# trzy/FasterRCNN

Measured on AMD Instinct MI355X. Metric: images/sec (600x1000) Faster-RCNN VGG-16 inference, higher is better.
Workload: dtype f32 (float32 tensors and accumulation; 15 GEMM layers in the f32x3 split-operand emulation = two fp16 terms per block-scaled operand, three fp16 MFMAs per product; 0 in f32x6 = three bf16 terms, six bf16 MFMAs; the other 2 on exact-f32 MFMA; strict exact-f32 everywhere: config.strict_f32_images_per_

## Files before the change

fasterrcnn_amd/_native.py:

```python
import ctypes as C
import os

_HERE = os.path.dirname(os.path.abspath(__file__))
LIB_PATH = os.environ.get("FRCNN_LIB_PATH") or os.path.join(_HERE, "csrc", "libfrcnn_hip.so")

OK = 0
ABI_VERSION = 21
ERRORS = {0: "FRCNN_OK", -1: "FRCNN_EINVAL", -2: "FRCNN_EHIP", -3: "FRCNN_ENOMEM",
          -4: "FRCNN_EUNSUPPORTED", -5: "FRCNN_ENODEVICE"}
RELU = 1
POOL2 = 2
NUM_KCLASS = 11
KCLASS_NAMES = ("conv3x3_mfma", "conv3x3_c3", "linear_mfma", "proposals", "roi_pool", "other", "winograd_transforms",
                "winograd_gemm", "winograd_x6_transforms", "winograd_x6_gemm", "winograd_x3f")

SYMBOLS = (
    "frcnn_abi_version", "frcnn_error_string", "frcnn_last_hip_error", "frcnn_device_count",
    "frcnn_anchors", "frcnn_pack_conv3x3", "frcnn_pack_conv3x3_c3", "frcnn_pack_fc_chw_to_hwc",
    "frcnn_pack_stack_rows", "frcnn_conv3x3_c3", "frcnn_conv3x3_c3_cmax", "frcnn_conv3x3_workspace_bytes", "frcnn_conv3x3_nhwc",
    "frcnn_maxpool2x2_nhwc",
    "frcnn_linear_workspace_bytes", "frcnn_linear", "frcnn_softmax_rows", "frcnn_rpn_proposals",
    "frcnn_nms", "frcnn_roi_pool", "frcnn_roi_pool_x3t", "frcnn_detections", "frcnn_ctx_create", "frcnn_ctx_create_proposals", "frcnn_ctx_destroy",
    "frcnn_ctx_bytes", "frcnn_vgg16_forward", "frcnn_ctx_tensor", "frcnn_ctx_timing_enable",
    "frcnn_ctx_timing_read",
    "frcnn_output_block_layout", "frcnn_stream_depend", "frcnn_ctx_submit_stats", "frcnn_predict_submit", "frcnn_streams_share_queue",
    "frcnn_fold_bn_pack", "frcnn_conv_workspace_bytes", "frcnn_conv_nhwc", "frcnn_conv_nhwc_math", "frcnn_conv_nhwc_x3g", "frcnn_conv_nhwc_x3g_tickets", "frcnn_pack_conv_x3g_weights", "frcnn_x3_saturation_events", "frcnn_tensor_absmax", "frcnn_conv7x7_s2_c3",
    "frcnn_maxpool3x3_s2_nhwc", "frcnn_spatial_mean_nhwc", "frcnn_resnet_forward", "frcnn_rpn_targets",
    "frcnn_preprocess_workspace_bytes", "frcnn_preprocess",
    "frcnn_conv3x3_uses_winograd", "frcnn_resnet_block_uses_winograd", "frcnn_pack_conv3x3_winograd",
    "frcnn_pack_conv3x3_winograd_taps", "frcnn_conv3x3_winograd_workspace_bytes",
    "frcnn_conv3x3_nhwc_winograd",
    "frcnn_conv3x3_uses_winograd_fused", "frcnn_resnet_block_uses_winograd_fused", "frcnn_pack_conv3x3_winograd_fused", "frcnn_pack_conv3x3_winograd_fused_taps",
    "frcnn_conv3x3_nhwc_winograd_fused",
    "frcnn_roi_align", "frcnn_roi_align_backward",
    "frcnn_x6t_record_bytes", "frcnn_split_rows_x6t", "frcnn_gemm_x6t_workspace_bytes", "frcnn_gemm_x6t", "frcnn_split_pixels_x6t", "frcnn_split_patches3x3_x6t",
    "frcnn_conv3x3_uses_winograd_x6", "frcnn_conv3x3_winograd_x6_pack_bytes", "frcnn_pack_conv3x3_winograd_x6",
    "frcnn_conv3x3_winograd_x6_workspace_bytes", "frcnn_conv3x3_nhwc_winograd_x6",
    "frcnn_pixel_absmax", "frcnn_split_pixels_x3t", "frcnn_split_patches3x3_x3t",
    "frcnn_x3t_blob_bytes", "frcnn_pack_rows_x3t", "frcnn_conv3x3_winograd_x3_pack_bytes", "frcnn_pack_conv3x3_winograd_x3",
    "frcnn_conv3x3_winograd_x3_workspace_bytes", "frcnn_conv3x3_nhwc_winograd_x3",
    "frcnn_conv3x3_winograd_x3_fused_workspace_bytes", "frcnn_conv3x3_nhwc_winograd_x3_fused", "frcnn_conv3x3_nhwc_winograd_x3_chain",
    "frcnn_x3t_record_bytes", "frcnn_rows_scale_x3t", "frcnn_split_rows_x3t", "frcnn_gemm_x3t_workspace_bytes", "frcnn_gemm_x3t",
    "frcnn_conv3x3_nhwc_winograd_fused_maps", "frcnn_ctx_create_backbone", "frcnn_resnet_backbone", "frcnn_resnet_forward_features", "frcnn_resnet_rpn_roipool", "frcnn_ctx_create_head", "frcnn_resnet_head",
    "frcnn_label_proposals", "frcnn_gather_rows", "frcnn_rpn_loss", "frcnn_detector_loss",
    "frcnn_gemm_tn_math", "frcnn_conv3x3_wgrad_math", "frcnn_conv_wgrad_math", "frcnn_bottleneck_backward_workspace_bytes", "frcnn_bottleneck_backward",
    "frcnn_gemm_tn_workspace_bytes", "frcnn_gemm_tn", "frcnn_conv3x3_wgrad_workspace_bytes", "frcnn_conv3x3_wgrad",
    "frcnn_pack_conv3x3_dgrad", "frcnn_relu_backward", "frcnn_dropout", "frcnn_dropout_relu_backward", "frcnn_add_inplace", "frcnn_maxpool2x2_backward",
    "frcnn_roi_pool_backward_workspace_bytes", "frcnn_roi_pool_backward", "frcnn_transpose", "frcnn_sgd_step", "frcnn_sgd_step_fold",
    "frcnn_conv_wgrad_workspace_bytes", "frcnn_conv_wgrad", "frcnn_conv_dgrad_workspace_bytes", "frcnn_conv_dgrad", "frcnn_conv_dgrad_math",
    "frcnn_pack_conv_dgrad", "frcnn_scale_rows", "frcnn_bn_scale_shift", "frcnn_spatial_mean_backward",
    "frcnn_ops_roi_align", "frcnn_ops_roi_align_backward", "frcnn_ops_roi_pool", "frcnn_ops_roi_pool_backward",
    "frcnn_ops_nms_workspace_bytes", "frcnn_ops_nms",
    "frcnn_ops_ms_roi_align", "frcnn_ops_ms_roi_align_workspace_bytes", "frcnn_ops_ms_roi_align_backward",
    "frcnn_ops_half_run", "frcnn_ops_roi_align_16", "frcnn_ops_roi_align_backward_16", "frcnn_ops_roi_pool_16",
    "frcnn_ops_roi_pool_backward_16", "frcnn_ops_ms_roi_align_16", "frcnn_ops_ms_roi_align_backward_16",
    "frcnn_ops_ps_roi_pool", "frcnn_ops_ps_roi_pool_backward", "frcnn_ops_ps_roi_align", "frcnn_ops_ps_roi_align_backward",
    "frcnn_ops_ps_roi_pool_16", "frcnn_ops_ps_roi_pool_backward_16", "frcnn_ops_ps_roi_align_16", "frcnn_ops_ps_roi_align_backward_16",
    "frcnn_ops_deform_workspace_bytes", "frcnn_ops_deform_forward", "frcnn_ops_deform_backward_columns", "frcnn_ops_deform_backward_offset",
    "frcnn_ops_deform_input_plan", "frcnn_ops_deform_backward_input", "frcnn_ops_deform_backward_weight",
    "frcnn_ops_deform_workspace_bytes_16", "frcnn_ops_deform_forward_16", "frcnn_ops_deform_backward_columns_16",
    "frcnn_ops_deform_backward_offset_16", "frcnn_ops_deform_input_plan_16", "frcnn_ops_deform_backward_input_16",
    "frcnn_ops_deform_backward_weight_16",
    "frcnn_ops_deform_roi_pool_cull_list", "frcnn_ops_deform_roi_pool_workspace_bytes", "frcnn_ops_deform_roi_pool",
    "frcnn_ops_deform_roi_pool_backward", "frcnn_ops_deform_roi_pool_16", "frcnn_ops_deform_roi_pool_backward_16",
    "frcnn_ops_box_iou_rotated", "frcnn_ops_nms_rotated", "frcnn_ops_roi_align_rotated_cull_list", "frcnn_ops_roi_align_rotated",
    "frcnn_ops_roi_align_rotated_backward", "frcnn_ops_roi_align_rotated_16", "frcnn_ops_roi_align_rotated_backward_16",
    "frcnn_ops_diff_iou_rotated", "frcnn_ops_diff_iou_rotated_backward",
    "frcnn_ops_convex_iou_tile_rows", "frcnn_ops_convex_iou", "frcnn_ops_convex_giou", "frcnn_ops_min_area_polygons",
    "frcnn_ops_soft_nms_block_threads", "frcnn_ops_soft_nms_lds_boxes", "frcnn_ops_soft_nms_max_boxes", "frcnn_ops_soft_nms_workspace_bytes",
    "frcnn_ops_soft_nms",
    "frcnn_ops_carafe_max_kernel", "frcnn_ops_carafe_channel_chunk", "frcnn_ops_carafe_tile_width", "frcnn_ops_carafe_tile_height",
    "frcnn_ops_carafe", "frcnn_ops_carafe_backward", "frcnn_ops_carafe_16", "frcnn_ops_carafe_backward_16",
    "frcnn_ops_msda_max_levels", "frcnn_ops_msda_max_points", "frcnn_ops_msda_max_channels", "frcnn_ops_msda_block_items",
    "frcnn_ops_msda_segment", "frcnn_ops_msda_workspace_bytes", "frcnn_ops_msda_forward", "frcnn_ops_msda_backward_loc", "frcnn_ops_msda_plan",
    "frcnn_ops_msda_backward_value", "frcnn_ops_msda_forward_16", "frcnn_ops_msda_backward_loc_16", "frcnn_ops_msda_backward_value_16",
    "frcnn_ops_prroi_pool_cull_list", "frcnn_ops_prroi_pool_workspace_bytes", "frcnn_ops_prroi_pool", "frcnn_ops_prroi_pool_backward",
    "frcnn_ops_prroi_pool_16", "frcnn_ops_prroi_pool_backward_16",
    "frcnn_ops_dcnv3_max_kernel", "frcnn_ops_dcnv3_max_channels", "frcnn_ops_dcnv3_block_items", "frcnn_ops_dcnv3_workspace_bytes",
    "frcnn_ops_dcnv3_forward", "frcnn_ops_dcnv3_backward_offset", "frcnn_ops_dcnv3_plan", "frcnn_ops_dcnv3_backward_input",
    "frcnn_ops_dcnv3_forward_16", "frcnn_ops_dcnv3_backward_offset_16", "frcnn_ops_dcnv3_backward_input_16",
    "frcnn_ops_dcnv4_record", "frcnn_ops_dcnv4_block_items", "frcnn_ops_dcnv4_workspace_bytes",
    "frcnn_ops_dcnv4_forward", "frcnn_ops_dcnv4_backward_offset_mask", "frcnn_ops_dcnv4_plan", "frcnn_ops_dcnv4_backward_input",
    "frcnn_ops_dcnv4_forward_16", "frcnn_ops_dcnv4_backward_offset_mask_16", "frcnn_ops_dcnv4_backward_input_16",
    "frcnn_ops_border_align_cull_list", "frcnn_ops_border_align", "frcnn_ops_border_align_backward", "frcnn_ops_border_align_16",
    "frcnn_ops_border_align_backward_16",
    "frcnn_ops_riroi_align_rotated_max_orientations", "frcnn_ops_riroi_align_rotated", "frcnn_ops_riroi_align_rotated_backward",
    "frcnn_ops_riroi_align_rotated_16", "frcnn_ops_riroi_align_rotated_backward_16",
    "frcnn_ops_rotated_feature_align", "frcnn_ops_rotated_feature_align_plan", "frcnn_ops_rotated_feature_align_backward",
    "frcnn_ops_rotated_feature_align_16", "frcnn_ops_rotated_feature_align_backward_16",
)


class FrcnnError(RuntimeError):
    def __init__(self, code, where, detail=""):
        self.code = code
        super().__init__("%s failed: %s (%d)%s" % (where, ERRORS.get(code, "?"), code,
                                                   (": " + detail) if detail else ""))


class VGG16Weights(C.Structure):
    _fields_ = [
        ("conv_w", C.c_void_p * 13), ("conv_b", C.c_void_p * 13),
        ("rpn_conv_w", C.c_void_p), ("rpn_conv_b", C.c_void_p),
        ("rpn_head_w", C.c_void_p), ("rpn_head_b", C.c_void_p),
# ... 190 lines not shown
    "frcnn_ops_convex_giou": (C.c_int, [_vp, _vp, _i, _vp, _vp, _vp]),
    "frcnn_ops_min_area_polygons": (C.c_int, [_vp, _i, _vp, _vp]),
    "frcnn_ops_soft_nms_block_threads": (C.c_int, []),
    "frcnn_ops_soft_nms_lds_boxes": (C.c_int, []),
    "frcnn_ops_soft_nms_max_boxes": (C.c_int, []),
    "frcnn_ops_soft_nms_workspace_bytes": (C.c_size_t, [_i]),
    "frcnn_ops_soft_nms": (C.c_int, [_vp, _vp, _vp, _vp, _i, _f, _f, _f, _i, _i, _vp, _vp, _vp, _sz, _vp]),
    "frcnn_ops_carafe_max_kernel": (C.c_int, []),
    "frcnn_ops_carafe_channel_chunk": (C.c_int, []),
    "frcnn_ops_carafe_tile_width": (C.c_int, []),
    "frcnn_ops_carafe_tile_height": (C.c_int, []),
    "frcnn_ops_carafe": (C.c_int, [_vp, _vp, _i, _i, _i, _i, _i, _i, _i, _vp, _vp]),
    "frcnn_ops_carafe_backward": (C.c_int, [_vp, _vp, _vp, _i, _i, _i, _i, _i, _i, _i, _vp, _vp, _vp]),
    "frcnn_ops_carafe_16": (C.c_int, [_i, _vp, _vp, _i, _i, _i, _i, _i, _i, _i, _vp, _vp]),
    "frcnn_ops_carafe_backward_16": (C.c_int, [_i, _vp, _vp, _vp, _i, _i, _i, _i, _i, _i, _i, _vp, _vp, _vp]),
    "frcnn_ops_msda_max_levels": (C.c_int, []),
    "frcnn_ops_msda_max_points": (C.c_int, []),
    "frcnn_ops_msda_max_channels": (C.c_int, []),
    "frcnn_ops_msda_block_items": (C.c_int, [_i, _i, _i, _i]),
    "frcnn_ops_msda_segment": (C.c_int, []),
    "frcnn_ops_msda_workspace_bytes": (C.c_size_t, [_i, _i, _i, _i, _i, _i, _i]),
    "frcnn_ops_msda_forward": (C.c_int, [_vp, _vp, _vp, _vp, _vp, _i, _i, _i, _i, _i, _i, _i, _vp, _vp]),
    "frcnn_ops_msda_backward_loc": (C.c_int, [_vp, _vp, _vp, _vp, _vp, _vp, _i, _i, _i, _i, _i, _i, _i, _vp, _vp, _vp]),
    "frcnn_ops_msda_plan": (C.c_int, [_vp, _vp, _vp, _vp, _i, _i, _i, _i, _i, _i, _vp, _vp, _vp]),
    "frcnn_ops_msda_backward_value": (C.c_int, [_vp, _vp, _vp, _vp, _i, _i, _i, _i, _i, _i, _i, _vp, _vp, _sz, _vp]),
    "frcnn_ops_msda_forward_16": (C.c_int, [_i, _vp, _vp, _vp, _vp, _vp, _i, _i, _i, _i, _i, _i, _i, _vp, _vp]),
    "frcnn_ops_msda_backward_loc_16": (C.c_int, [_i, _vp, _vp, _vp, _vp, _vp, _vp, _i, _i, _i, _i, _i, _i, _i, _vp, _vp, _vp]),
    "frcnn_ops_msda_backward_value_16": (C.c_int, [_i, _vp, _vp, _vp, _vp, _i, _i, _i, _i, _i, _i, _i, _vp, _vp, _sz, _vp]),
    "frcnn_ops_prroi_pool_cull_list": (C.c_int, []),
    "frcnn_ops_prroi_pool_workspace_bytes": (C.c_size_t, [_i, _i, _i]),
    "frcnn_ops_prroi_pool": (C.c_int, [_vp, _i, _i, _i, _i, _vp, _i, _i, _i, _f, _vp, _vp]),
    "frcnn_ops_prroi_pool_backward": (C.c_int, [_vp, _vp, _i, _i, _i, _i, _i, _i, _i, _f, _vp, _vp, _vp, _vp, _sz, _vp]),
    "frcnn_ops_prroi_pool_16": (C.c_int, [_i, _vp, _i, _i, _i, _i, _vp, _i, _i, _i, _f, _vp, _vp]),
    "frcnn_ops_prroi_pool_backward_16": (C.c_int, [_i, _vp, _vp, _i, _i, _i, _i, _i, _i, _i, _f, _vp, _vp, _vp, _vp, _sz, _vp]),
    "frcnn_ops_border_align_cull_list": (C.c_int, []),
    "frcnn_ops_border_align": (C.c_int, [_vp, _i, _i, _i, _i, _vp, _i, _i, _vp, _vp, _vp]),
    "frcnn_ops_border_align_backward": (C.c_int, [_vp, _i, _i, _i, _i, _i, _i, _vp, _vp, _vp, _vp]),
    "frcnn_ops_border_align_16": (C.c_int, [_i, _vp, _i, _i, _i, _i, _vp, _i, _i, _vp, _vp, _vp]),
    "frcnn_ops_border_align_backward_16": (C.c_int, [_i, _vp, _i, _i, _i, _i, _i, _i, _vp, _vp, _vp, _vp]),
    "frcnn_ops_rotated_feature_align": (C.c_int, [_vp, _vp, _i, _i, _i, _i, _f, _i, _vp, _vp]),
    "frcnn_ops_rotated_feature_align_plan": (C.c_int, [_vp, _i, _i, _i, _f, _i, _vp, _vp, _vp]),
    "frcnn_ops_rotated_feature_align_backward": (C.c_int, [_vp, _vp, _vp, _vp, _i, _i, _i, _i, _i, _vp, _vp]),
    "frcnn_ops_rotated_feature_align_16": (C.c_int, [_i, _vp, _vp, _i, _i, _i, _i, _f, _i, _vp, _vp]),
    "frcnn_ops_rotated_feature_align_backward_16": (C.c_int, [_i, _vp, _vp, _vp, _vp, _i, _i, _i, _i, _i, _vp, _vp]),
    "frcnn_ops_dcnv3_max_kernel": (C.c_int, []),
    "frcnn_ops_dcnv3_max_channels": (C.c_int, []),
    "frcnn_ops_dcnv3_block_items": (C.c_int, [_i, _i, _i, _i]),
    "frcnn_ops_dcnv3_workspace_bytes": (C.c_size_t, [_i] * 13),
    "frcnn_ops_dcnv3_forward": (C.c_int, [_vp, _vp, _vp] + [_i] * 13 + [_f, _vp, _vp]),
    "frcnn_ops_dcnv3_backward_offset": (C.c_int, [_vp, _vp, _vp, _vp] + [_i] * 13 + [_f, _vp, _vp, _vp]),
    "frcnn_ops_dcnv3_plan": (C.c_int, [_vp, _vp] + [_i] * 12 + [_f, _vp, _vp, _vp]),
    "frcnn_ops_dcnv3_backward_input": (C.c_int, [_vp, _vp, _vp, _vp] + [_i] * 13 + [_vp, _vp, _sz, _vp]),
    "frcnn_ops_dcnv3_forward_16": (C.c_int, [_i, _vp, _vp, _vp] + [_i] * 13 + [_f, _vp, _vp]),
    "frcnn_ops_dcnv3_backward_offset_16": (C.c_int, [_i, _vp, _vp, _vp, _vp] + [_i] * 13 + [_f, _vp, _vp, _vp]),
    "frcnn_ops_dcnv3_backward_input_16": (C.c_int, [_i, _vp, _vp, _vp, _vp] + [_i] * 13 + [_vp, _vp, _sz, _vp]),
    "frcnn_ops_dcnv4_record": (C.c_int, [_i, _i, _i, _i]),
    "frcnn_ops_dcnv4_block_items": (C.c_int, [_i, _i, _i, _i, _i]),
    "frcnn_ops_dcnv4_workspace_bytes": (C.c_size_t, [_i] * 14),
    "frcnn_ops_dcnv4_forward": (C.c_int, [_vp, _vp] + [_i] * 13 + [_f, _i, _vp, _vp]),
    "frcnn_ops_dcnv4_backward_offset_mask": (C.c_int, [_vp, _vp, _vp] + [_i] * 13 + [_f, _i, _vp, _vp]),
    "frcnn_ops_dcnv4_plan": (C.c_int, [_vp] + [_i] * 12 + [_f, _i, _vp, _vp, _vp]),
    "frcnn_ops_dcnv4_backward_input": (C.c_int, [_vp, _vp, _vp, _vp] + [_i] * 14 + [_vp, _vp, _sz, _vp]),
    "frcnn_ops_dcnv4_forward_16": (C.c_int, [_i, _vp, _vp] + [_i] * 13 + [_f, _i, _vp, _vp]),
    "frcnn_ops_dcnv4_backward_offset_mask_16": (C.c_int, [_i, _vp, _vp, _vp] + [_i] * 13 + [_f, _i, _vp, _vp]),
    "frcnn_ops_dcnv4_backward_input_16": (C.c_int, [_i, _vp, _vp, _vp, _vp] + [_i] * 14 + [_vp, _vp, _sz, _vp]),
    "frcnn_x6t_record_bytes": (C.c_size_t, [_i, _i]),
    "frcnn_split_rows_x6t": (C.c_int, [_vp, _i, _sz, _vp, _i, _i, _i, _i, _vp]),
    "frcnn_gemm_x6t_workspace_bytes": (C.c_size_t, [_i, _i, _i, _i]),
    "frcnn_gemm_x6t": (C.c_int, [_vp, _i, _sz, _vp, _i, _sz, _vp, _vp, _vp, _i, _sz, _i, _i, _i, _i, _u, _vp, _sz, _vp]),
    "frcnn_split_pixels_x6t": (C.c_int, [_vp, _vp, _i, _i, _i, _i, _i, _i, _vp]),
    "frcnn_conv3x3_uses_winograd_x6": (C.c_int, [_i, _i]),
    "frcnn_conv3x3_winograd_x6_pack_bytes": (C.c_size_t, [_i, _i]),
    "frcnn_pack_conv3x3_winograd_x6": (C.c_int, [_vp, _vp, _vp, _i, _i, _vp]),
    "frcnn_conv3x3_winograd_x6_workspace_bytes": (C.c_size_t, [_i, _i, _i, _i, _i]),
    "frcnn_conv3x3_nhwc_winograd_x6": (C.c_int, [_vp, _vp, _vp, _vp, _i, _i, _i, _i, _i, _u, _vp, _sz, _vp]),
    "frcnn_split_patches3x3_x6t": (C.c_int, [_vp, _vp, _i, _i, _i, _i, _i, _i, _vp]),
    "frcnn_conv3x3_uses_winograd_fused": (C.c_int, [_i, _i]),
    "frcnn_resnet_block_uses_winograd_fused": (C.c_int, [_i, _i, _i]),
    "frcnn_pack_conv3x3_winograd_fused": (C.c_int, [_vp, _vp, _vp, _i, _i, _vp]),
    "frcnn_pack_conv3x3_winograd_fused_taps": (C.c_int, [_vp, _vp, _i, _i, _i, _vp]),
    "frcnn_conv3x3_nhwc_winograd_fused": (C.c_int, [_vp, _vp, _vp, _vp, _i, _i, _i, _i, _u, _vp]),
    "frcnn_linear_workspace_bytes": (C.c_size_t, [_i, _i, _i]),
    "frcnn_linear": (C.c_int, [_vp, _i, _vp, _vp, _vp, _i, _i, _i, _i, _u, _vp, _sz, _vp]),
    "frcnn_softmax_rows": (C.c_int, [_vp, _i, _vp, _i, _i, _vp]),
    "frcnn_rpn_proposals": (C.c_int, [_vp, _vp, _i, _vp, _vp, _i, _i, _i, _i, _i, _i, _f, _f,
                                      _vp, _vp, _vp, _vp, _vp]),
    "frcnn_nms": (C.c_int, [_vp, _vp, _vp, _i, _f, _i, _vp, _vp, _vp]),
    "frcnn_roi_pool": (C.c_int, [_vp, _i, _i, _i, _vp, _vp, _i, _i, _f, _vp, _vp]),
    "frcnn_roi_pool_x3t": (C.c_int, [_vp, _i, _i, _i, _vp, _vp, _i, _i, _f, _vp, _vp, _vp, _i, _vp]),
    "frcnn_detections": (C.c_int, [_vp, _vp, _vp, _vp, _i, _i, _i, _i, _f, _f, _vp, _vp, _vp]),
    "frcnn_ctx_create": (C.c_int, [C.POINTER(C.c_void_p), _i, _i, _i]),
    "frcnn_ctx_create_proposals": (C.c_int, [C.POINTER(C.c_void_p), _i, _i]),
    "frcnn_ctx_destroy": (None, [_vp]),
    "frcnn_ctx_bytes": (C.c_size_t, [_vp]),
    "frcnn_vgg16_forward": (C.c_int, [_vp, C.POINTER(VGG16Weights), C.POINTER(ForwardParams), _vp, _i, _i,
                                      _vp, _vp, _vp, _vp, _vp, _vp, _vp]),
    "frcnn_ctx_tensor": (C.c_int, [_vp, _i, C.POINTER(C.c_void_p), C.POINTER(C.c_size_t)]),
    "frcnn_rpn_targets": (C.c_int, [_vp, _vp, _i, _vp, _i, C.c_double, C.c_double, _vp, _vp, _vp, _vp, _vp, _vp]),
    "frcnn_preprocess_workspace_bytes": (C.c_size_t, [_i, _i, _i, _i]),
    "frcnn_preprocess": (C.c_int, [_vp, _i, _i, _i, _i, _i, _i, _f, C.POINTER(C.c_float), C.POINTER(C.c_float), _vp, _vp,
                                   _vp, _sz, _vp]),
    "frcnn_fold_bn_pack": (C.c_int, [_vp, _vp, _vp, _vp, _vp, _f, _i, _i, _i, _vp, _vp, _vp]),
    "frcnn_conv_workspace_bytes": (C.c_size_t, [_i, _i, _i, _i, _i, _i, _i, _i]),
    "frcnn_conv_nhwc": (C.c_int, [_vp, _vp, _vp, _vp, _vp, _i, _i, _i, _i, _i, _i, _i, _i, _u, _vp, _sz, _vp]),
    "frcnn_x3_saturation_events": (C.c_int, [C.POINTER(C.c_ulonglong)]),
    "frcnn_conv_nhwc_math": (C.c_int, [_vp, _vp, _vp, _vp, _vp, _i, _i, _i, _i, _i, _i, _i, _i, _u, _i, _vp, _sz, _vp]),
    "frcnn_conv_nhwc_x3g": (C.c_int, [_vp, _vp, _vp, _vp, _vp, _i, _i, _i, _i, _i, _i, _i, _i, _u, _vp, _vp, _vp, _vp, _sz, _vp]),
    "frcnn_conv_nhwc_x3g_tickets": (C.c_int, [_vp, _vp, _vp, _vp, _vp, _i, _i, _i, _i, _i, _i, _i, _i, _u, _vp, _vp, _vp, _vp, _sz, _vp, _vp]),
    "frcnn_pack_conv_x3g_weights": (C.c_int, [_vp, _vp, _vp, _i, _i, _i, _vp]),
    "frcnn_tensor_absmax": (C.c_int, [_vp, C.c_longlong, _vp, _vp]),
    "frcnn_conv7x7_s2_c3": (C.c_int, [_vp, _vp, _vp, _vp, _i, _i, _i, _u, _vp]),
    "frcnn_maxpool3x3_s2_nhwc": (C.c_int, [_vp, _vp, _i, _i, _i, _vp]),
    "frcnn_spatial_mean_nhwc": (C.c_int, [_vp, _vp, _i, _i, _i, _i, _vp]),
    "frcnn_resnet_forward": (C.c_int, [_vp, C.POINTER(ResNetWeights), C.POINTER(ForwardParams), _vp, _i, _i,
                                       _vp, _vp, _vp, _vp, _vp, _vp, _vp]),
    "frcnn_resnet_forward_features": (C.c_int, [_vp, C.POINTER(ResNetWeights), C.POINTER(ForwardParams), _vp, _i, _i,
                                                _vp, _vp, _vp, _vp, _vp, _vp, _vp]),
    "frcnn_resnet_backbone": (C.c_int, [_vp, C.POINTER(ResNetWeights), C.POINTER(ForwardParams), _vp, _i, _i, _i, _vp, _vp]),
    "frcnn_pixel_absmax": (C.c_int, [_vp, _vp, C.c_longlong, _i, _vp]),
    "frcnn_split_pixels_x3t": (C.c_int, [_vp, _vp, _vp, _vp, _i, _i, _i, _i, _i, _i, _vp]),
    "frcnn_split_patches3x3_x3t": (C.c_int, [_vp, _vp, _vp, _vp, _i, _i, _i, _i, _i, _i, _vp]),
    "frcnn_x3t_blob_bytes": (C.c_size_t, [_i, _i, _i]),
    "frcnn_pack_rows_x3t": (C.c_int, [_vp, _i, _sz, _vp, _i, _i, _i, _i, _vp]),
    "frcnn_conv3x3_winograd_x3_pack_bytes": (C.c_size_t, [_i, _i]),
    "frcnn_pack_conv3x3_winograd_x3": (C.c_int, [_vp, _vp, _i, _i, _vp]),
    "frcnn_conv3x3_winograd_x3_workspace_bytes": (C.c_size_t, [_i, _i, _i, _i, _i]),
    "frcnn_conv3x3_nhwc_winograd_x3": (C.c_int, [_vp, _vp, _vp, _vp, _i, _i, _i, _i, _i, _u, _vp, _sz, _vp]),
    "frcnn_conv3x3_winograd_x3_fused_workspace_bytes": (C.c_size_t, [_i, _i, _i]),
    "frcnn_conv3x3_nhwc_winograd_x3_fused": (C.c_int, [_vp, _vp, _vp, _vp, _i, _i, _i, _i, _i, _u, _vp, _sz, _vp]),
    "frcnn_conv3x3_nhwc_winograd_x3_chain": (C.c_int, [_vp, _vp, _vp, _vp, _i, _i, _i, _i, _i, _u, _i, _vp, _sz, _vp, _vp, _vp]),
    "frcnn_x3t_record_bytes": (C.c_size_t, [_i, _i]),
    "frcnn_rows_scale_x3t": (C.c_int, [_vp, _i, _sz, _vp, _i, _i, _i, _i, _vp]),
    "frcnn_split_rows_x3t": (C.c_int, [_vp, _i, _sz, _vp, _vp, _i, _i, _i, _i, _vp]),
    "frcnn_gemm_x3t_workspace_bytes": (C.c_size_t, [_i, _i, _i, _i]),
    "frcnn_gemm_x3t": (C.c_int, [_vp, _vp, _i, _sz, _sz, _vp, _vp, _i, _sz, _sz, _vp, _vp, _vp, _i, _sz, _i, _i, _i, _i, _u, _vp, _sz, _vp]),
    "frcnn_ctx_create_backbone": (C.c_int, [C.POINTER(C.c_void_p), _i, _i, _i]),
    "frcnn_ctx_create_head": (C.c_int, [C.POINTER(C.c_void_p), _i]),
    "frcnn_resnet_rpn_roipool": (C.c_int, [_vp, C.POINTER(ResNetWeights), C.POINTER(ForwardParams), _vp, _i, _i, _vp, _vp, _vp, _vp, _vp, _vp]),
    "frcnn_resnet_head": (C.c_int, [_vp, C.POINTER(ResNetWeights), C.POINTER(ForwardParams), _vp, _i, _vp, _vp, _vp]),
    "frcnn_conv3x3_nhwc_winograd_fused_maps": (C.c_int, [_vp, _vp, _vp, _vp, _i, _i, _i, _i, _i, _u, _vp]),
    "frcnn_label_proposals": (C.c_int, [_vp, _vp, _i, _vp, _vp, _i, _i, _f, _f, C.POINTER(C.c_float), C.POINTER(C.c_float),
                                        _vp, _vp, _vp, _vp, _vp, _vp]),
    "frcnn_gather_rows": (C.c_int, [_vp, _vp, _i, _i, _vp, _vp]),
    "frcnn_rpn_loss": (C.c_int, [_vp, _i, _i, _vp, _i, _vp, _vp, _vp, _vp]),
    "frcnn_detector_loss": (C.c_int, [_vp, _vp, _vp, _vp, _i, _i, _vp, _vp, _i, _vp]),
    "frcnn_gemm_tn_workspace_bytes": (C.c_size_t, [_i, _i, _i]),
    "frcnn_gemm_tn": (C.c_int, [_vp, _i, _vp, _i, _vp, _i, _i, _i, _i, _vp, _sz, _vp]),
    "frcnn_gemm_tn_math": (C.c_int, [_vp, _i, _vp, _i, _vp, _i, _i, _i, _i, _i, _vp, _sz, _vp]),
    "frcnn_conv3x3_wgrad_math": (C.c_int, [_vp, _vp, _vp, _i, _i, _i, _i, _i, _vp, _sz, _vp]),
    "frcnn_conv_wgrad_math": (C.c_int, [_vp, _vp, _vp, _i, _i, _i, _i, _i, _i, _i, _i, _i, _vp, _sz, _vp]),
    "frcnn_bottleneck_backward_workspace_bytes": (C.c_int, [_vp, _vp, _vp, _vp, _i, _i, _i, _i, _i, C.POINTER(C.c_size_t), C.POINTER(C.c_size_t)]),
    "frcnn_bottleneck_backward": (C.c_int, [_vp, _vp, _vp, _vp, _vp, _vp, _vp, _vp, _vp, _vp, _vp, _vp, _vp, _i, _i, _i, _i, _i, _i, _vp, _sz, _vp, _sz,
                                            _vp, _vp]),
    "frcnn_conv3x3_wgrad_workspace_bytes": (C.c_size_t, [_i, _i, _i, _i]),
    "frcnn_conv3x3_wgrad": (C.c_int, [_vp, _vp, _vp, _i, _i, _i, _i, _vp, _sz, _vp]),
    "frcnn_pack_conv3x3_dgrad": (C.c_int, [_vp, _vp, _i, _i, _vp]),
    "frcnn_conv_wgrad_workspace_bytes": (C.c_size_t, [_i] * 8),
    "frcnn_conv_wgrad": (C.c_int, [_vp, _vp, _vp, _i, _i, _i, _i, _i, _i, _i, _i, _vp, _sz, _vp]),
    "frcnn_conv_dgrad_workspace_bytes": (C.c_size_t, [_i] * 8),
    "frcnn_conv_dgrad": (C.c_int, [_vp, _vp, _vp, _vp, _i, _i, _i, _i, _i, _i, _i, _i, _vp, _sz, _vp]),
    "frcnn_conv_dgrad_math": (C.c_int, [_vp, _vp, _vp, _vp, _i, _i, _i, _i, _i, _i, _i, _i, _i, _vp, _sz, _vp]),
    "frcnn_pack_conv_dgrad": (C.c_int, [_vp, _vp, _i, _i, _i, _vp]),
    "frcnn_scale_rows": (C.c_int, [_vp, _vp, _vp, _i, _i, _i, _vp]),
    "frcnn_bn_scale_shift": (C.c_int, [_vp, _vp, _vp, _vp, _f, _i, _vp, _vp, _vp]),
    "frcnn_spatial_mean_backward": (C.c_int, [_vp, _vp, _i, _i, _i, _i, _vp]),
    "frcnn_relu_backward": (C.c_int, [_vp, _vp, _sz, _vp]),
# ... 87 lines not shown
```

fasterrcnn_amd/csrc/api.hip:

```cpp
#include "common.h"
#include <algorithm>
#include <cmath>
#include <cstring>
#include <initializer_list>
#include <string>
#include <vector>
#include <new>

namespace frcnn {

static thread_local std::string g_hip_error;
void set_hip_error(hipError_t e) { g_hip_error = hipGetErrorString(e); }

static size_t align_up(size_t v, size_t a) { return (v + a - 1) / a * a; }

struct EventRec { int cls; hipEvent_t start, stop; };

struct Scratch {
    void* p = nullptr;
    size_t bytes = 0;
    int reserve(size_t want, hipStream_t s, bool zero)
    {
        if (want <= bytes) return FRCNN_OK;
        if (p) { FRCNN_HIP_TRY(hipStreamSynchronize(s)); release(); }
// ... 467 lines not shown

int frcnn_conv_nhwc_math(const float* d_x, const float* d_wp, const float* d_bias, const float* d_residual, float* d_y,
                         int N, int H, int W, int cin, int cout, int ksize, int stride, int pad, unsigned flags, int math,
                         void* d_ws, size_t ws_bytes, void* stream)
{
    if (!d_x || !d_wp || !d_bias || !d_y) return FRCNN_EINVAL;
    if (flags & FRCNN_POOL2) return FRCNN_EUNSUPPORTED;
    return launch_conv_gather(d_x, d_wp, d_bias, d_residual, d_y, N, H, W, cin, cout, ksize, stride, pad, flags,
                              d_ws, ws_bytes, as_stream(stream), math);
}

int frcnn_x3_saturation_events(unsigned long long* out)
{
    if (!out) return FRCNN_EINVAL;
    const unsigned* c = x3_saturation_counter();
    *out = c ? (unsigned long long)*reinterpret_cast<const volatile unsigned*>(c) : 0ull;
    return FRCNN_OK;
}

int frcnn_conv_nhwc_x3g(const float* d_x, const float* d_wp, const float* d_bias, const float* d_residual, float* d_y,
                        int N, int H, int W, int cin, int cout, int ksize, int stride, int pad, unsigned flags,
                        const float* d_xmax, const float* d_wmax, float* d_ymax, void* d_ws, size_t ws_bytes, void* stream)
{
    if (!d_x || !d_wp || !d_bias || !d_y || !d_xmax || !d_wmax) return FRCNN_EINVAL;
    if (flags & FRCNN_POOL2) return FRCNN_EUNSUPPORTED;
    const GatherX3 x3{d_xmax, d_wmax, d_ymax, nullptr, (flags & FRCNN_X3G_WSPLIT) != 0};
    return launch_conv_gather(d_x, d_wp, d_bias, d_residual, d_y, N, H, W, cin, cout, ksize, stride, pad, flags,
                              d_ws, ws_bytes, as_stream(stream), FRCNN_CONV_F32X3G, &x3);
}

int frcnn_pack_conv_x3g_weights(const float* d_wp, const float* d_wmax, void* d_out, int taps, int cout, int cin, void* stream)
{
    if (taps < 1 || cout < 1) return FRCNN_EINVAL;
    return launch_pack_x3g_weights(d_wp, d_wmax, d_out, (long long)taps * cout, cin, as_stream(stream));
}

int frcnn_conv_nhwc_x3g_tickets(const float* d_x, const float* d_wp, const float* d_bias, const float* d_residual, float* d_y,
                                int N, int H, int W, int cin, int cout, int ksize, int stride, int pad, unsigned flags,
                                const float* d_xmax, const float* d_wmax, float* d_ymax, void* d_ws, size_t ws_bytes,
                                unsigned* d_tile_counters, void* stream)
{
    static_assert(FRCNN_X3G_TILE_COUNTERS == GX_TILE_COUNTERS, "one bound on both sides of the ABI");
    if (!d_x || !d_wp || !d_bias || !d_y || !d_xmax || !d_wmax || !d_tile_counters) return FRCNN_EINVAL;
    if (flags & FRCNN_POOL2) return FRCNN_EUNSUPPORTED;
    const GatherX3 x3{d_xmax, d_wmax, d_ymax, d_tile_counters, (flags & FRCNN_X3G_WSPLIT) != 0};
    return launch_conv_gather(d_x, d_wp, d_bias, d_residual, d_y, N, H, W, cin, cout, ksize, stride, pad, flags,
                              d_ws, ws_bytes, as_stream(stream), FRCNN_CONV_F32X3G, &x3);
}

int frcnn_tensor_absmax(const float* d_x, long long n, float* d_out, void* stream)
{
    if (!d_x || !d_out) return FRCNN_EINVAL;
    return launch_tensor_absmax(d_x, n, d_out, as_stream(stream));
}

int frcnn_conv7x7_s2_c3(const float* d_x, const float* d_wp, const float* d_bias, float* d_y, int H, int W,
                        int cout, unsigned flags, void* stream)
{
    if (!d_x || !d_wp || !d_bias || !d_y) return FRCNN_EINVAL;
    return launch_conv7x7_s2_c3(d_x, d_wp, d_bias, d_y, H, W, cout, flags, as_stream(stream));
}

int frcnn_maxpool3x3_s2_nhwc(const float* d_x, float* d_y, int H, int W, int c, void* stream)
{
    if (!d_x || !d_y) return FRCNN_EINVAL;
    return launch_maxpool3x3_s2(d_x, d_y, H, W, c, as_stream(stream));
}

int frcnn_spatial_mean_nhwc(const float* d_x, float* d_y, int N, int H, int W, int c, void* stream)
{
    if (!d_x || !d_y) return FRCNN_EINVAL;
    return launch_spatial_mean(d_x, d_y, N, H, W, c, as_stream(stream));
}

size_t frcnn_linear_workspace_bytes(int M, int N, int K) { return linear_workspace_bytes(M, N, K); }

int frcnn_linear(const float* d_a, int lda, const float* d_w, const float* d_bias, float* d_y, int ldy,
                 int M, int N, int K, unsigned flags, void* d_ws, size_t ws_bytes, void* stream)
{
    if (!d_a || !d_w || !d_bias || !d_y) return FRCNN_EINVAL;
    return launch_linear(d_a, lda, d_w, d_bias, d_y, ldy, M, N, K, flags, d_ws, ws_bytes, as_stream(stream));
}

int frcnn_softmax_rows(const float* d_x, int ldx, float* d_y, int M, int ncls, void* stream)
{
    if (!d_x || !d_y) return FRCNN_EINVAL;
    return launch_softmax_rows(d_x, ldx, d_y, M, ncls, as_stream(stream));
}

int frcnn_rpn_proposals(frcnn_ctx* ctx, const float* d_head, int ld_head, const float* d_anchor_map,
                        const float* d_valid_map, int fh, int fw, int image_h, int image_w, int pre_nms,
                        int post_nms, float nms_threshold, float min_side, float* d_scores,
                        int32_t* d_sorted_idx, float* d_props, int32_t* d_counts, void* stream)
{
    if (!ctx || !d_head || !d_anchor_map || !d_scores || !d_sorted_idx || !d_props || !d_counts) return FRCNN_EINVAL;
    FRCNN_HIP_TRY(hipMemsetAsync(d_counts, 0, 4 * sizeof(int32_t), as_stream(stream)));
    return launch_rpn_proposals(ctx->ps, d_head, ld_head, d_anchor_map, d_valid_map, fh, fw, image_h, image_w,
                                pre_nms, post_nms, nms_threshold, min_side, d_scores, d_sorted_idx, d_props,
                                d_counts, as_stream(stream));
}

int frcnn_nms(frcnn_ctx* ctx, const float* d_boxes, const float* d_scores, int n, float threshold,
              int max_keep, int32_t* d_keep, int32_t* d_n_keep, void* stream)
{
    if (!ctx || !d_boxes || !d_scores || !d_keep || !d_n_keep) return FRCNN_EINVAL;
    return launch_nms(ctx->ps, d_boxes, d_scores, n, threshold, max_keep, d_keep, d_n_keep, as_stream(stream));
}

int frcnn_roi_pool(const float* d_fm, int fh, int fw, int c, const float* d_rois, const int32_t* d_n_rois,
                   int max_rois, int pooled, float spatial_scale, float* d_out, void* stream)
{
    if (!d_fm || !d_rois || !d_n_rois || !d_out) return FRCNN_EINVAL;
    return launch_roi_pool(d_fm, fh, fw, c, d_rois, d_n_rois, max_rois, pooled, spatial_scale, d_out,
                           as_stream(stream));
}

int frcnn_roi_pool_x3t(const float* d_fm, int fh, int fw, int c, const float* d_rois, const int32_t* d_n_rois, int max_rois, int pooled,
                       float spatial_scale, float* d_cmax, float* d_inv_scale, void* d_rec, int rec_rows, void* stream)
{
    if (!d_fm || !d_rois || !d_n_rois || !d_cmax || !d_inv_scale || !d_rec) return FRCNN_EINVAL;
    return launch_roi_pool_x3t(d_fm, fh, fw, c, d_rois, d_n_rois, max_rois, pooled, spatial_scale, d_cmax, d_inv_scale, d_rec, rec_rows,
                               as_stream(stream));
}

int frcnn_roi_align(const float* d_fm, int fh, int fw, int c, const float* d_rois, const int32_t* d_n_rois, int max_rois,
                    int pooled, float spatial_scale, int sampling_ratio, int aligned, float* d_out, void* stream)
{
    if (!d_fm || !d_rois || !d_n_rois || !d_out) return FRCNN_EINVAL;
    return launch_roi_align(d_fm, fh, fw, c, d_rois, d_n_rois, max_rois, pooled, spatial_scale, sampling_ratio, aligned, d_out,
                            as_stream(stream));
}

int frcnn_roi_align_backward(const float* d_rois, int n_rois, int fh, int fw, int c, int pooled, float spatial_scale,
                             int sampling_ratio, int aligned, const float* d_dout, float* d_dfm, int accumulate, void* stream)
{
    if (!d_dfm || (n_rois > 0 && (!d_rois || !d_dout))) return FRCNN_EINVAL;
    return launch_roi_align_backward(d_rois, n_rois, fh, fw, c, pooled, spatial_scale, sampling_ratio, aligned, d_dout, d_dfm,
                                     accumulate, as_stream(stream));
}

int frcnn_detections(const float* d_props, const float* d_classes, const float* d_deltas,
                     const int32_t* d_n_rois, int max_rois, int ncls, int image_h, int image_w,
                     float score_threshold, float nms_threshold, double* d_out, int32_t* d_out_cnt, void* stream)
{
    if (!d_props || !d_classes || !d_deltas || !d_n_rois || !d_out || !d_out_cnt) return FRCNN_EINVAL;
    return launch_detections(d_props, d_classes, d_deltas, d_n_rois, max_rois, ncls, image_h, image_w,
                             score_threshold, nms_threshold, d_out, d_out_cnt, as_stream(stream));
}

int frcnn_label_proposals(const float* d_props, const int32_t* d_n_props, int max_props,
                          const float* d_gt_boxes, const int32_t* d_gt_class_idx, int n_gt, int num_classes,
                          float min_background_iou, float min_object_iou,
                          const float box_delta_means[4], const float box_delta_stds[4],
                          float* d_out_props, int32_t* d_out_class_idx, float* d_out_gt_classes,
                          float* d_out_gt_box_deltas, int32_t* d_out_count, void* stream)
{
    if ((!d_props && max_props > 0) || !d_n_props || !d_gt_boxes || !d_gt_class_idx || !box_delta_means || !box_delta_stds ||
        !d_out_props || !d_out_class_idx || !d_out_gt_classes || !d_out_gt_box_deltas || !d_out_count)
        return FRCNN_EINVAL;
    if (!(min_background_iou < min_object_iou)) return FRCNN_EINVAL;
    return launch_label_proposals(d_props, d_n_props, max_props, d_gt_boxes, d_gt_class_idx, n_gt, num_classes,
                                  min_background_iou, min_object_iou, box_delta_means, box_delta_stds, d_out_props,
                                  d_out_class_idx, d_out_gt_classes, d_out_gt_box_deltas, d_out_count, as_stream(stream));
}

int frcnn_gather_rows(const float* d_src, const int32_t* d_idx, int n, int row_floats, float* d_dst, void* stream)
// ... 492 lines not shown
}

int run_wino_x6_layer(frcnn_ctx* c, const float* x, const void* urec, const float* b, float* y, int h, int w, int ci, int co,
                      unsigned flags, hipStream_t s, int N = 1)
{
    if (N == 1 && !conv3x3_uses_winograd_x6(ci, co)) return FRCNN_EINVAL;
    int r = ensure_wx_ws(c, conv3x3_winograd_x6_workspace_bytes(N, h, w, ci, co), s);
    if (r) return r;
    void *V = nullptr, *G = nullptr;
    float* M = nullptr;
    size_t gb = 0;
    r = winograd_x6_plan(N, h, w, ci, co, flags, c->wx_ws.p, c->wx_ws.bytes, &V, &M, &G, &gb);
    if (r) return r;
    { Scope _t(c, 8, s); r = launch_winograd_x6_input(x, V, N, h, w, ci, s); }
    if (r) return r;
    { Scope _g(c, 9, s); r = launch_winograd_x6_gemm(V, urec, M, N, h, w, ci, co, G, gb, s); }
    if (r) return r;
    Scope _o(c, 8, s);
    return launch_winograd_output(M, b, y, N, h, w, co, flags, s);
}

int run_wino_x3_layer(frcnn_ctx* c, const float* x, const void* ublob, const float* b, float* y, int h, int w, int ci, int co,
                      unsigned flags, hipStream_t s, int N = 1, const float* cmax_ready = nullptr, float* cmax_out = nullptr)
{
    if (N == 1 && !conv3x3_uses_winograd_x6(ci, co)) return FRCNN_EINVAL;
    int r = ensure_wx_ws(c, conv3x3_winograd_x3_workspace_bytes(N, h, w, ci, co), s);
    if (r) return r;
    void *V = nullptr, *G = nullptr;
    float *M = nullptr, *vinv = nullptr, *cmax = nullptr;
    size_t gb = 0;
    r = winograd_x3_plan(N, h, w, ci, co, flags, c->wx_ws.p, c->wx_ws.bytes, &V, &vinv, &cmax, &M, &G, &gb);
    if (r) return r;
    { Scope _t(c, 8, s); r = launch_winograd_x3_input(x, cmax, V, vinv, N, h, w, ci, s, cmax_ready); }
    if (r) return r;
    { Scope _g(c, 9, s); r = launch_winograd_x3_gemm(V, vinv, ublob, M, N, h, w, ci, co, G, gb, s); }
    if (r) return r;
    Scope _o(c, 8, s);
    return launch_winograd_output(M, b, y, N, h, w, co, flags, s, cmax_out);
}

int ensure_x3f_cmax(frcnn_ctx* c, size_t need, hipStream_t s)
{
    return c->x3f_cmax.reserve(3 * std::max(need, (size_t)c->max_h * c->max_w * sizeof(float)), s, false);
}
size_t x3f_cmax_bytes(const frcnn_ctx* c) { return c->x3f_cmax.bytes / 3; }
float* x3f_cmax_buffer(frcnn_ctx* c, int which) { return reinterpret_cast<float*>(static_cast<unsigned char*>(c->x3f_cmax.p) + (size_t)which * x3f_cmax_bytes(c)); }

int run_wino_x3f_layer(frcnn_ctx* c, const float* x, const void* ublob, const float* b, float* y, int h, int w, int ci, int co,
                       unsigned flags, hipStream_t s, const float* cmax_ready = nullptr, float* cmax_out = nullptr)
{
    int r = ensure_x3f_cmax(c, conv3x3_winograd_x3_fused_workspace_bytes(1, h, w), s);
    if (r) return r;
    Scope _w(c, 10, s);
    return launch_conv3x3_winograd_x3_fused(x, ublob, b, y, 1, h, w, ci, co, flags, x3f_cmax_buffer(c, 0), x3f_cmax_bytes(c), s, cmax_ready, cmax_out);
}

int run_wino_fused_layer(frcnn_ctx* c, bool , const float* x, const float* u, const float* b, float* y, int h, int w, int ci,
                         int co, unsigned flags, hipStream_t s, int n_maps = 1)
{
    Scope _w(c, 7, s);
    return launch_conv3x3_winograd_fused(x, u, b, y, h, w, ci, co, flags, s, n_maps);
}

struct BlocksTargetScope {
    explicit BlocksTargetScope(int t, int wino_rows = 0, int x6_tiles = 0) { conv3x3_set_blocks_target(t); linear_batched_set_tile(wino_rows); gemm_x6t_set_tiles(x6_tiles); }
    ~BlocksTargetScope() { conv3x3_set_blocks_target(0); linear_batched_set_tile(0); gemm_x6t_set_tiles(0); }
};

int check_forward_params(const frcnn_forward_params* p, int bad_math_mode)
{
    if ((p->winograd_x3_mask & ~p->winograd_x6_mask) != 0) return FRCNN_EINVAL;
    if (p->math_mode != FRCNN_MATH_F32 && p->math_mode != FRCNN_MATH_F32_WINOGRAD) return bad_math_mode;
    if ((p->roi_op != FRCNN_ROI_POOL && p->roi_op != FRCNN_ROI_ALIGN) || p->roi_sampling_ratio > 2) return FRCNN_EINVAL;
    if (p->conv_blocks_target < 0) return FRCNN_EINVAL;
    if (p->winograd_tile_rows != 0 && p->winograd_tile_rows != 64 && p->winograd_tile_rows != 128) return FRCNN_EINVAL;
    if (p->x6_gemm_tiles < 0 || p->x6_gemm_tiles > 2) return FRCNN_EINVAL;
    return FRCNN_OK;
}

int run_rpn_after_trunk(frcnn_ctx* c, const float* head_w, const float* head_b, const frcnn_forward_params* p, int H, int W, int fh, int fw,
                        int C, const float* d_anchor_map, const float* d_valid_map, float* d_props, int32_t* d_counts, hipStream_t s)
{
    int rc;
    STEP(2, launch_linear(c->rpn_trunk, C, head_w, head_b, c->rpn_head, 128, fh * fw, 45, C, 0u, c->lin_ws, c->lin_ws_bytes, s));
    const float* amap = d_anchor_map;
    const float* vmap = d_valid_map;
    if (!amap || !vmap) {
        if (c->anc_h != H || c->anc_w != W || c->anc_fh != fh || c->anc_fw != fw) {
            STEP(5, launch_anchors(H, W, fh, fw, 16, c->anchor_map, c->valid_map, s));
            c->anc_h = H; c->anc_w = W; c->anc_fh = fh; c->anc_fw = fw;
        }
        amap = c->anchor_map; vmap = c->valid_map;
    }
    FRCNN_HIP_TRY(hipMemsetAsync(d_counts, 0, 4 * sizeof(int32_t), s));
    STEP(3, launch_rpn_proposals(c->ps, c->rpn_head, 128, amap, p->allow_edge_proposals ? nullptr : vmap, fh, fw,
                                 H, W, p->pre_nms, p->post_nms, p->rpn_nms_threshold, p->min_side, c->scores,
                                 c->sorted_idx, d_props, d_counts, s));
    return FRCNN_OK;
}

int run_roi_f32(frcnn_ctx* c, const frcnn_forward_params* p, int fh, int fw, int C, const float* d_props, const int32_t* d_counts,
                float* dst, hipStream_t s)
{
    Scope _sc(c, 4, s);
    if (p->roi_op == FRCNN_ROI_ALIGN)
        return launch_roi_align(c->fm, fh, fw, C, d_props, d_counts + 2, p->post_nms, 7, 1.0f / 16.0f, p->roi_sampling_ratio, 0, dst, s);
    return launch_roi_pool(c->fm, fh, fw, C, d_props, d_counts + 2, p->post_nms, 7, 1.0f / 16.0f, dst, s);
}

int run_detector_heads(frcnn_ctx* c, const float* head_w, const float* head_b, int ncls, int V, int n_rois, float* d_classes,
                       float* d_deltas, hipStream_t s)
{
    int rc;
    const int nd = (ncls - 1) * 4;
    const int hld = cdiv(ncls + nd, 128) * 128;
    c->last_head_ld = hld;
    STEP(2, launch_linear(c->fc2_out, V, head_w, head_b, c->head_logits, hld, n_rois, ncls + nd, V, 0u, c->lin_ws, c->lin_ws_bytes, s));
    STEP(5, launch_head_finish(c->head_logits, hld, n_rois, ncls, nd, d_classes, d_deltas, s));
    return FRCNN_OK;
}
}

int frcnn_vgg16_forward(frcnn_ctx* c, const frcnn_vgg16_weights* w, const frcnn_forward_params* p,
                        const float* d_image, int H, int W, const float* d_anchor_map,
                        const float* d_valid_map, float* d_props, float* d_classes, float* d_deltas,
                        int32_t* d_counts, void* stream)
{
    if (!c || !w || !p || !d_image || !d_props || !d_classes || !d_deltas || !d_counts) return FRCNN_EINVAL;
    if (H < 16 || W < 16 || H > c->max_h || W > c->max_w) return FRCNN_EINVAL;
    if (p->post_nms < 1 || p->post_nms > c->max_rois || p->pre_nms < 1 || p->pre_nms > c->pre_cap) return FRCNN_EINVAL;
    if (w->num_classes < 2 || w->num_classes > FRCNN_MAX_NUM_CLASSES) return FRCNN_EUNSUPPORTED;
    for (int i = 0; i < 13; ++i) if (!w->conv_w[i] || !w->conv_b[i]) return FRCNN_EINVAL;
    if (!w->rpn_conv_w || !w->rpn_conv_b || !w->rpn_head_w || !w->rpn_head_b || !w->fc1_w || !w->fc1_b ||
        !w->fc2_w || !w->fc2_b || !w->head_w || !w->head_b)
        return FRCNN_EINVAL;
    hipStream_t s = as_stream(stream);
    const unsigned R = FRCNN_RELU, RP = FRCNN_RELU | FRCNN_POOL2;
    int rc = check_forward_params(p, FRCNN_EINVAL);
    if (rc) return rc;
    if (p->fc_math_mode != FRCNN_FC_F32 && p->fc_math_mode != FRCNN_FC_F32X6T && p->fc_math_mode != FRCNN_FC_F32X3T) return FRCNN_EINVAL;
    BlocksTargetScope target_scope(p->conv_blocks_target, p->winograd_tile_rows, p->x6_gemm_tiles);
    const bool wino = p->math_mode == FRCNN_MATH_F32_WINOGRAD;
    if (p->winograd_x6_mask != 0 && (!wino || (p->winograd_x6_mask & ~0x3FFE) != 0)) return FRCNN_EINVAL;
    if (p->winograd_x3f_mask != 0 && (!wino || (p->winograd_x3f_mask & ~0x3FFE) != 0 || (p->winograd_x3f_mask & p->winograd_x6_mask) != 0)) return FRCNN_EINVAL;
    int layer_index = 0;
    const float* cmax_ready = nullptr;
    size_t cmax_used = 0, cmax_cleared = 0;
    if (wino && ((p->winograd_x3f_mask | (p->winograd_x3_mask & p->winograd_x6_mask)) & 0x1FFE) != 0) {
        int r0 = ensure_x3f_cmax(c, (size_t)H * W * sizeof(float), s);
        if (r0) return r0;
        static const int co_of[13] = {0, 64, 128, 128, 256, 256, 256, 512, 512, 512, 512, 512, 512};
        static const bool pool_of[13] = {false, true, false, true, false, false, true, false, false, true, false, false, false};
        size_t want = 0;
        int eh = H, ew = W;
        for (int li = 1; li <= 12; ++li) {
            const bool f3 = ((p->winograd_x3f_mask >> li) & 1) != 0;
            const bool t3 = !f3 && ((p->winograd_x6_mask >> li) & 1) && ((p->winograd_x3_mask >> li) & 1);
            const unsigned efl = FRCNN_RELU | (pool_of[li] ? FRCNN_POOL2 : 0u);
            if (pool_of[li]) { eh /= 2; ew /= 2; }
            if ((f3 || t3) && (f3 || winograd_output_emits_cmax(co_of[li], efl))) want += ((size_t)eh * ew + 63) & ~(size_t)63;
        }
        if (want > 2 * x3f_cmax_bytes(c) / sizeof(float)) return FRCNN_EINVAL;
        cmax_cleared = want;
        if (want) FRCNN_HIP_TRY(hipMemsetAsync(x3f_cmax_buffer(c, 1), 0, cmax_cleared * sizeof(float), s));
    }
    auto conv3 = [&](const float* xin, const float* wgt, const float* bs, float* yout, int hh, int ww, int ci, int co,
                     unsigned fl) -> int {
        ++layer_index;
        const float* in_cmax = cmax_ready;
        cmax_ready = nullptr;
        const bool is_x3f = wino && ((p->winograd_x3f_mask >> layer_index) & 1);
        const bool is_x3 = wino && !is_x3f && ((p->winograd_x6_mask >> layer_index) & 1) && ((p->winograd_x3_mask >> layer_index) & 1);
        float* out_cmax = nullptr;
        if ((is_x3f || is_x3) && layer_index != FRCNN_X6_RPN_TRUNK_BIT && (fl & FRCNN_RELU) && (is_x3f || winograd_output_emits_cmax(co, fl))) {
            const int oh = (fl & FRCNN_POOL2) ? hh / 2 : hh, ow = (fl & FRCNN_POOL2) ? ww / 2 : ww;
            const size_t need = ((size_t)oh * ow + 63) & ~(size_t)63;
            out_cmax = x3f_cmax_buffer(c, 1) + cmax_used;
            cmax_used += need;
            if (cmax_used > cmax_cleared) return FRCNN_EINVAL;
        }
        int r1;
        if (is_x3f)
            r1 = run_wino_x3f_layer(c, xin, wgt, bs, yout, hh, ww, ci, co, fl, s, in_cmax, out_cmax);
        else if (is_x3)
            r1 = run_wino_x3_layer(c, xin, wgt, bs, yout, hh, ww, ci, co, fl, s, 1, in_cmax, out_cmax);
        else if (wino && ((p->winograd_x6_mask >> layer_index) & 1))
            r1 = run_wino_x6_layer(c, xin, wgt, bs, yout, hh, ww, ci, co, fl, s);
        else
            r1 = -9999;
        if (r1 != -9999) {
            if (r1 == FRCNN_OK) cmax_ready = out_cmax;
            return r1;
        }
        if (wino && conv3x3_uses_winograd_fused(ci, co)) {
            return run_wino_fused_layer(c, p->conv_blocks_target == 0, xin, wgt, bs, yout, hh, ww, ci, co, fl, s);
        }
        Scope _d(c, 0, s);
        return launch_conv3x3_nhwc(xin, wgt, bs, yout, hh, ww, ci, co, fl, c->conv_ws, c->conv_ws_bytes, s);
    };
#define CONV(call) do { rc = (call); } while (0); if (rc) return rc

// ... 610 lines not shown
```

fasterrcnn_amd/csrc/common.h:

```cpp
#pragma once
#include <hip/hip_runtime.h>
#include <stdint.h>
#include <stddef.h>
#include <stdlib.h>
#include "../../include/frcnn_hip.h"

typedef float f32x4  __attribute__((ext_vector_type(4)));
typedef float f32x16 __attribute__((ext_vector_type(16)));

inline const char* frcnn_knob(const char* name)
{
#ifdef FRCNN_EXPERIMENT_KNOBS
    return getenv(name);
#else
    (void)name;
    return nullptr;
#endif
}

namespace frcnn {

void set_hip_error(hipError_t e);

inline int check_launch() {
    hipError_t e = hipGetLastError();
    if (e != hipSuccess) { set_hip_error(e); return FRCNN_EHIP; }
    return FRCNN_OK;
}

#define FRCNN_HIP_TRY(expr)                                   \
    do {                                                      \
        hipError_t _e = (expr);                               \
        if (_e != hipSuccess) { ::frcnn::set_hip_error(_e); return FRCNN_EHIP; } \
    } while (0)

static inline int cdiv(int a, int b) { return (a + b - 1) / b; }

struct DeviceOnce { unsigned char done[64]; };
inline int set_max_dynamic_lds(DeviceOnce& once, const void* kern, size_t bytes)
{
    int dev = 0;
    FRCNN_HIP_TRY(hipGetDevice(&dev));
    if (dev < 0 || dev >= 64) return FRCNN_EINVAL;
    if (!once.done[dev]) {
        FRCNN_HIP_TRY(hipFuncSetAttribute(kern, hipFuncAttributeMaxDynamicSharedMemorySize, (int)bytes));
        once.done[dev] = 1;
    }
    return FRCNN_OK;
}
#define FRCNN_MAX_LDS_ONCE(kern, bytes)                                                                  \
    do {                                                                                                 \
        static ::frcnn::DeviceOnce _once = {};                                                           \
        const int _rc = ::frcnn::set_max_dynamic_lds(_once, reinterpret_cast<const void*>(kern), (bytes)); \
        if (_rc) return _rc;                                                                             \
    } while (0)

static inline bool conv3x3_uses_winograd(int cin, int cout) { return cin >= 128 && cout >= 256 && cin % 16 == 0 && cout % 128 == 0; }
static inline bool resnet_block_uses_winograd(int width, int stride) { return stride == 1 && width >= 256 && width % 128 == 0; }

struct KernelTimer;

}

namespace frcnn {

int launch_anchors(int image_h, int image_w, int fh, int fw, int feature_pixels,
                   float* anchor_map, float* valid_map, hipStream_t s);

int launch_pack_conv3x3(const float* w, float* wp, int cout, int cin, hipStream_t s);
int launch_pack_conv3x3_c3(const float* w, float* wp, int cout, hipStream_t s);
int launch_pack_fc_chw_to_hwc(const float* w, float* wp, int out_f, int c, int phw, hipStream_t s);
int launch_pack_stack_rows(const float* w1, const float* b1, int n1, const float* w2, const float* b2,
                           int n2, int k, int n_pad, float* wo, float* bo, hipStream_t s);

int launch_conv3x3_c3(const float* x, const float* wp, const float* b, float* y, int H, int W,
                      int cout, unsigned flags, hipStream_t s, float* cmax_out = nullptr);
size_t conv3x3_workspace_bytes(int H, int W, int cin, int cout);
int conv3x3_blocks_target();
void conv3x3_set_blocks_target(int target);
int launch_conv3x3_nhwc(const float* x, const float* wp, const float* b, float* y, int H, int W,
                        int cin, int cout, unsigned flags, void* ws, size_t ws_bytes, hipStream_t s);
int launch_maxpool2x2(const float* x, float* y, int H, int W, int c, hipStream_t s);

size_t conv_gather_workspace_bytes(int N, int H, int W, int cin, int cout, int R, int stride, int pad);
#define FRCNN_CONV_F32X3G 2
static constexpr int GX_TILE_COUNTERS = 16384;
struct GatherX3 { const float* xmax; const float* wmax; float* ymax; unsigned* tile_counters = nullptr; bool wsplit = false; bool trusted = false; };
int launch_pack_x3g_weights(const float* wp, const float* wmax, void* out, long long rows, int cin, hipStream_t s);
int launch_conv_gather(const float* x, const float* wp, const float* bias, const float* residual, float* y,
                       int N, int H, int W, int cin, int cout, int R, int stride, int pad, unsigned flags,
                       void* ws, size_t ws_bytes, hipStream_t s, int math = FRCNN_GRAD_F32, const GatherX3* x3 = nullptr);
unsigned* x3_saturation_counter();
int launch_tensor_absmax(const float* x, long long n, float* out, hipStream_t s);
int launch_conv7x7_s2_c3(const float* x, const float* wp, const float* b, float* y, int H, int W, int cout,
                         unsigned flags, hipStream_t s);
int launch_maxpool3x3_s2(const float* x, float* y, int H, int W, int c, hipStream_t s);
int launch_spatial_mean(const float* x, float* y, int N, int H, int W, int c, hipStream_t s);
int launch_fold_bn_pack(const float* w, const float* gamma, const float* beta, const float* mean, const float* var,
                        float eps, int cout, int cin, int ksize, float* wp, float* bp, hipStream_t s);

size_t linear_workspace_bytes(int M, int N, int K);
int launch_linear(const float* a, int lda, const float* w, const float* bias, float* y, int ldy,
                  int M, int N, int K, unsigned flags, void* ws, size_t ws_bytes, hipStream_t s);
int launch_linear_batched(const float* a, int lda, size_t a_stride, const float* w, size_t w_stride, float* y, int ldy,
                          size_t y_stride, int M, int N, int K, int batches, hipStream_t s);
void linear_batched_set_tile(int rows);
size_t conv3x3_winograd_workspace_bytes(int N, int H, int W, int cin, int cout);
int launch_pack_conv3x3_winograd(const float* w, const float* scale, float* u, int cout, int cin, hipStream_t s);
int launch_pack_conv3x3_winograd_taps(const float* wp, float* u, int cout, int cin, int data_gradient, hipStream_t s);
int launch_conv3x3_winograd(const float* x, const float* u, const float* b, float* y, int N, int H, int W, int cin, int cout,
                            unsigned flags, void* ws, size_t ws_bytes, hipStream_t s);
int winograd_plan(int N, int H, int W, int cin, int cout, unsigned flags, void* ws, size_t ws_bytes, float** V, float** M);
int launch_winograd_input(const float* x, float* V, int N, int H, int W, int cin, hipStream_t s);
int launch_winograd_gemm(const float* V, const float* u, float* M, int N, int H, int W, int cin, int cout, hipStream_t s);
int launch_winograd_output(const float* M, const float* b, float* y, int N, int H, int W, int cout, unsigned flags, hipStream_t s,
                           float* cmax_out = nullptr);
bool winograd_output_emits_cmax(int cout, unsigned flags);
static inline bool conv3x3_uses_winograd_fused(int cin, int cout) { return cin >= 64 && cin % 16 == 0 && cout >= 64 && cout % 64 == 0; }
static inline bool resnet_block_uses_winograd_fused(int n_maps, int width, int stride)
{
    return n_maps == 1 && stride == 1 && conv3x3_uses_winograd_fused(width, width);
}
bool conv3x3_winograd_fused_ok(int H, int W, int cin, int cout);
int launch_pack_conv3x3_winograd_fused(const float* w, const float* scale, float* u, int cout, int cin, hipStream_t s);
int launch_pack_conv3x3_winograd_fused_taps(const float* wp, float* u, int cout, int cin, int data_gradient, hipStream_t s);
int launch_conv3x3_winograd_fused(const float* x, const float* u, const float* b, float* y, int H, int W, int cin, int cout,
                                  unsigned flags, hipStream_t s, int n_maps = 1);
int gemm_x6t_row_tile(int M);
int gemm_x6t_col_tile(int N);
size_t x6t_record_bytes(int rows_padded, int K);
int launch_split_rows_x6t(const float* a, int lda, size_t a_batch_floats, void* rec, int R, int rows_padded, int K, int batches, hipStream_t s);
bool gemm_x6t_shape_ok(int M, int N, int K, int batches);
size_t gemm_x6t_workspace_bytes(int M, int N, int K, int batches);
void gemm_x6t_set_tiles(int mode);
int launch_gemm_x6t(const void* a_rec, int a_rows, size_t a_batch_bytes, const void* b_rec, int b_rows, size_t b_batch_bytes,
                    const float* bias, const float* residual, float* c, int ldc, size_t c_batch_floats, int M, int N, int K, int batches,
                    unsigned flags, void* ws, size_t ws_bytes, hipStream_t s, int tiles_mode = -1);
int launch_split_pixels_x6t(const float* x, void* rec, int N, int H, int W, int C, int stride, int rows_padded, hipStream_t s);
int gemm_x6t_get_tiles();
int launch_gemm_x6t_reduce(const float* ws, const float* bias, const float* residual, float* c, int ldc, size_t c_batch_floats, int M, int N,
                           int batches, int splits, int relu, hipStream_t s);
size_t x3t_record_bytes(int rows_padded, int K);
int launch_rows_scale_x3t(const float* a, int lda, size_t a_batch_floats, float* inv_scale, int R, int rows_padded, int K, int batches,
                          hipStream_t s);
int launch_split_rows_x3t(const float* a, int lda, size_t a_batch_floats, const float* inv_scale, void* rec, int R, int rows_padded, int K,
                          int batches, hipStream_t s);
int launch_split_pixels_x3t(const float* x, const float* cmax, void* rec, float* inv, int N, int H, int W, int C, int stride, int rows_padded,
                            hipStream_t s);
int launch_split_patches3x3_x3t(const float* x, const float* cmax, void* rec, float* inv, int N, int H, int W, int C, int stride,
                                int rows_padded, hipStream_t s);
size_t gemm_x3t_workspace_bytes(int M, int N, int K, int batches);
int launch_gemm_x3t(const void* a_rec, const float* a_inv, int a_rows, size_t a_batch_bytes, size_t a_inv_batch, const void* b_rec,
                    const float* b_inv, int b_rows, size_t b_batch_bytes, size_t b_inv_batch, const float* bias, const float* residual,
                    float* c, int ldc, size_t c_batch_floats, int M, int N, int K, int batches, unsigned flags, void* ws, size_t ws_bytes,
                    hipStream_t s, int tiles_mode = -1);
size_t x3t_blob_bytes(int rows_padded, int K, int batches);
int launch_pack_rows_x3t(const float* a, int lda, size_t a_batch_floats, void* blob, int R, int rows_padded, int K, int batches, hipStream_t s);
int launch_pixel_absmax(const float* x, float* cmax, long long pixels, int C, hipStream_t s);
size_t conv3x3_winograd_x3_pack_bytes(int cout, int cin);
int launch_pack_conv3x3_winograd_x3(const float* u_f32, void* ublob, int cout, int cin, hipStream_t s);
size_t conv3x3_winograd_x3_workspace_bytes(int N, int H, int W, int cin, int cout);
int winograd_x3_plan(int N, int H, int W, int cin, int cout, unsigned flags, void* ws, size_t ws_bytes, void** V, float** vinv, float** cmax,
                     float** M, void** G, size_t* g_bytes);
int launch_winograd_x3_input(const float* x, float* cmax, void* vrec, float* vinv, int N, int H, int W, int cin, hipStream_t s,
                             const float* cmax_ready = nullptr);
int launch_winograd_x3_gemm(const void* vrec, const float* vinv, const void* ublob, float* M, int N, int H, int W, int cin, int cout, void* gws,
                            size_t gws_bytes, hipStream_t s);
int launch_conv3x3_winograd_x3(const float* x, const void* ublob, const float* b, float* y, int N, int H, int W, int cin, int cout,
                               unsigned flags, void* ws, size_t ws_bytes, hipStream_t s,
                               const float* cmax_ready = nullptr, float* cmax_out = nullptr);
size_t conv3x3_winograd_x3_fused_workspace_bytes(int N, int H, int W);
int launch_conv3x3_winograd_x3_fused(const float* x, const void* ublob, const float* b, float* y, int N, int H, int W, int cin, int cout,
                                     unsigned flags, void* ws, size_t ws_bytes, hipStream_t s, const float* cmax_ready = nullptr,
                                     float* cmax_out = nullptr);
int launch_roi_pool_x3t(const float* fm, int fh, int fw, int c, const float* rois, const int32_t* n_rois, int max_rois, int pooled,
                        float scale, float* cmax, float* inv, void* rec, int rec_rows, hipStream_t s, bool cmax_ready = false);
bool conv3x3_uses_winograd_x6(int cin, int cout);
size_t conv3x3_winograd_x6_pack_bytes(int cout, int cin);
size_t conv3x3_winograd_x6_workspace_bytes(int N, int H, int W, int cin, int cout);
int launch_pack_conv3x3_winograd_x6(const float* w, const float* scale, void* urec, int cout, int cin, hipStream_t s);
int launch_winograd_x6_input(const float* x, void* vrec, int N, int H, int W, int cin, hipStream_t s);
int launch_winograd_x6_gemm(const void* vrec, const void* urec, float* M, int N, int H, int W, int cin, int cout, void* gws, size_t gws_bytes, hipStream_t s);
int winograd_x6_plan(int N, int H, int W, int cin, int cout, unsigned flags, void* ws, size_t ws_bytes, void** V, float** M, void** G, size_t* g_bytes);
int launch_conv3x3_winograd_x6(const float* x, const void* urec, const float* b, float* y, int N, int H, int W, int cin, int cout,
                               unsigned flags, void* ws, size_t ws_bytes, hipStream_t s);
int launch_split_patches3x3_x6t(const float* x, void* rec, int N, int H, int W, int C, int stride, int rows_padded, hipStream_t s);
int launch_softmax_rows(const float* x, int ldx, float* y, int M, int ncls, hipStream_t s);
int launch_head_finish(const float* x, int ldx, int M, int ncls, int ndelta, float* classes,
                       float* deltas, hipStream_t s);

struct ProposalScratch {
    unsigned long long* keys;
    float*    boxes_all;
    float*    cand_boxes;
    float*    cand_scores;
    unsigned long long* mask;
    int32_t*  keep;
    int       a_cap, pre_cap, post_cap;
};
size_t proposal_scratch_bytes(int a_cap, int pre_cap, int post_cap);
void   proposal_scratch_carve(ProposalScratch& ps, void* base, int a_cap, int pre_cap, int post_cap);

int launch_rpn_proposals(const ProposalScratch& ps, const float* head, int ld_head,
                         const float* anchor_map, const float* valid_map, int fh, int fw,
                         int image_h, int image_w, int pre_nms, int post_nms, float nms_thr,
                         float min_side, float* scores, int32_t* sorted_idx, float* props,
                         int32_t* counts, hipStream_t s);
int launch_nms(const ProposalScratch& ps, const float* boxes, const float* scores, int n, float thr,
               int max_keep, int32_t* keep, int32_t* n_keep, hipStream_t s);

int launch_roi_pool(const float* fm, int fh, int fw, int c, const float* rois, const int32_t* n_rois,
                    int max_rois, int pooled, float scale, float* out, hipStream_t s);
int launch_roi_pool_x6t(const float* fm, int fh, int fw, int c, const float* rois, const int32_t* n_rois,
                        int max_rois, int pooled, float scale, void* rec, int rec_rows, hipStream_t s);

int launch_roi_align(const float* fm, int fh, int fw, int c, const float* rois, const int32_t* n_rois, int max_rois, int pooled,
                     float scale, int sampling_ratio, int aligned, float* out, hipStream_t s);
int launch_roi_align_backward(const float* rois, int n_rois, int fh, int fw, int c, int pooled, float scale, int sampling_ratio,
                              int aligned, const float* dout, float* dfm, int accumulate, hipStream_t s);

int launch_rpn_targets(const float* anchor_map, const float* valid_map, int A, const float* gt, int M,
                       double obj_thr, double bg_thr, float* rpn_map, int32_t* obj_idx, int32_t* bg_idx,
                       int32_t* counts, void* ws, hipStream_t s);

size_t preprocess_workspace_bytes(int H, int W, int Ho, int Wo);
int launch_preprocess(const unsigned char* rgb, int H, int W, int Ho, int Wo, int bgr, int flip, float scaling,
                      const float* means, const float* stds, float* out, unsigned char* out_u8, void* ws,
                      size_t ws_bytes, hipStream_t s);

int launch_detections(const float* props, const float* classes, const float* deltas,
                      const int32_t* n_rois, int max_rois, int ncls, int image_h, int image_w,
                      float score_thr, float nms_thr, double* out, int32_t* out_cnt, hipStream_t s);

size_t gemm_tn_workspace_bytes(int M, int N, int R, int taps);
int launch_gemm_tn(const float* A, int lda, const float* B, int ldb, float* C, int ldc, int M, int N, int R,
                   void* ws, size_t ws_bytes, hipStream_t s, int math = FRCNN_GRAD_F32);
int launch_conv3x3_wgrad(const float* x, const float* dz, float* dwp, int H, int W, int cin, int cout,
                         void* ws, size_t ws_bytes, hipStream_t s, int math = FRCNN_GRAD_F32);
int gemm_nt16_splits(int M, int N, int R);
size_t gemm_nt16_workspace_bytes(int M, int N, int R);
int launch_gemm_nt16(int elem_type, const void* A, int lda, const void* B, int ldb, float* C, int ldc, int M, int N, int R, hipStream_t s);
int launch_gemm_nt16_split(int elem_type, const void* A, int lda, const void* B, int ldb, float* C, int ldc, int M, int N, int R,
                           int accumulate, void* ws, size_t ws_bytes, hipStream_t s);
int launch_gemm_nt16_nchw(int elem_type, const void* A, int lda, const void* B, int ldb, int M, int N, int R, const void* bias, void* out,
                          int P, int c_total, int c_base, hipStream_t s);
int launch_label_proposals(const float* props, const int32_t* n_props, int max_props, const float* gt,
                           const int32_t* gt_cls, int M, int ncls, float bg_thr, float obj_thr,
                           const float means[4], const float stds[4], float* out_props, int32_t* out_cls,
                           float* out_onehot, float* out_deltas, int32_t* out_count, hipStream_t s);
int launch_gather_rows(const float* src, const int32_t* idx, int n, int row_floats, float* dst, hipStream_t s);
int launch_rpn_loss(const float* head, int ld, int cells, const int32_t* sample, int n_sample, const float* rpn_map,
                    float* losses, float* d_head, hipStream_t s);
int launch_detector_loss(const float* classes, const float* deltas, const float* gt_onehot, const float* gt_deltas,
                         int S, int ncls, float* losses, float* d_logits, int ld, hipStream_t s);
int launch_relu_backward(float* dy, const float* y, size_t n, hipStream_t s);
int launch_dropout(float* x, size_t n, float p, float scale, const uint64_t* seed, uint32_t stream_id, uint32_t rank,
                   uint8_t* keep_out, hipStream_t s);
int launch_dropout_relu_backward(float* dy, const float* y, size_t n, float scale, hipStream_t s);
int launch_add_inplace(float* a, const float* b, size_t n, hipStream_t s);
int launch_maxpool2x2_backward(const float* x, const float* dy, float* dx, int H, int W, int C, hipStream_t s);
size_t roi_pool_backward_workspace_bytes(int n_rois, int pooled, int C);
int launch_roi_pool_backward(const float* fm, int fh, int fw, int C, const float* rois, int n_rois, int pooled,
                             float scale, const float* dout, float* dfm, int accumulate, void* ws, size_t ws_bytes,
                             hipStream_t s);
int launch_transpose(const float* x, int ldi, float* y, int ldo, int rows, int cols, hipStream_t s);
int launch_pack_conv3x3_dgrad(const float* wp, float* wd, int cout, int cin, hipStream_t s);
int launch_conv_wgrad(const float* x, const float* dz, float* dwp, int N, int H, int W, int cin, int cout, int ks, int stride,
                      int pad, void* ws, size_t ws_bytes, hipStream_t s, int math = FRCNN_GRAD_F32);
size_t conv_dgrad_workspace_bytes(int N, int H, int W, int cin, int cout, int R, int stride, int pad);
int launch_conv_dgrad(const float* dz, const float* wd, const float* residual, float* dx, int N, int H, int W, int cin,
                      int cout, int R, int stride, int pad, void* ws, size_t ws_bytes, hipStream_t s, int math = FRCNN_GRAD_F32);
int launch_pack_conv_dgrad(const float* wp, float* wd, int taps, int cout, int cin, hipStream_t s);
int launch_scale_rows(const float* src, const float* scale, float* dst, int taps, int cout, int cin, hipStream_t s);
int launch_bn_scale_shift(const float* gamma, const float* beta, const float* mean, const float* var, float eps, int c,
                          float* scale, float* shift, hipStream_t s);
int launch_spatial_mean_backward(const float* dy, float* dx, int N, int H, int W, int c, hipStream_t s);
int launch_sgd(float* w, const float* g, float* buf, size_t n, float lr, float momentum, float weight_decay, int first,
               hipStream_t s);
int launch_sgd_fold(float* w, const float* g, float* buf, size_t n, float lr, float momentum, float weight_decay, int first,
                    const float* scale, float* folded, int cout, int cin, hipStream_t s);

}
```

fasterrcnn_amd/csrc/linear.hip:

```cpp
#include "common.h"
#include <cstdlib>

namespace frcnn {

static constexpr int LLDK = 20;

template <int TM, int TN, int WM, int WN>
struct GemmCfg {
    static constexpr int BM = 32 * TM * WM;
    static constexpr int BN = 32 * TN * WN;
    static constexpr int THREADS = 64 * WM * WN;
    static constexpr int NA = (BM * 4 + THREADS - 1) / THREADS;
    static constexpr int NB = (BN * 4 + THREADS - 1) / THREADS;
    static constexpr int A_F = BM * LLDK;
    static constexpr int B_F = BN * LLDK;
    static constexpr size_t LDS_BYTES = (size_t)2 * (A_F + B_F) * sizeof(float);
    static_assert(THREADS == 256 || THREADS == 512, "4 or 8 waves per block");
};

struct BatchGeom { long long a_stride, w_stride, y_stride; int nblocks, mblocks, batches; };

template <int TM, int TN, int WM, int WN, bool BATCHED, int NSETS = 2>
__global__ __launch_bounds__(64 * WM * WN)
void linear_mfma_kernel(const float* __restrict__ a, int lda, const float* __restrict__ w,
// ... 150 lines not shown
            for (int s = 0; s < nst; ++s) stage(s, areg[0], breg[0]);
        }
    }

    const bool direct = (gridDim.z == 1);
    float* const dst = direct ? y : ws + (size_t)blockIdx.z * M * N;
    const int ldd = direct ? ldy : N;
#pragma unroll
    for (int j = 0; j < TN; ++j) {
        const int n = n0 + 32 * (TN * wn + j) + li;
        if (n >= N) continue;
        const float bv = (direct && bias != nullptr) ? bias[n] : 0.f;
#pragma unroll
        for (int i = 0; i < TM; ++i) {
#pragma unroll
            for (int r = 0; r < 16; ++r) {
                const int m = m0 + 32 * (TM * wm + i) + (r & 3) + 8 * (r >> 2) + 4 * lh;
                if (m < M) {
                    float v = acc[i][j][r] + bv;
                    if (direct && relu) v = fmaxf(v, 0.f);
                    dst[(size_t)m * ldd + n] = v;
                }
            }
        }
    }
}

__global__ __launch_bounds__(256)
void splitk_reduce_kernel(const float* __restrict__ ws, const float* __restrict__ bias,
                          float* __restrict__ y, int ldy, int M, int N, int splits, int relu)
{
    const size_t total = (size_t)M * N;
    for (size_t i = (size_t)blockIdx.x * 256 + threadIdx.x; i < total; i += (size_t)gridDim.x * 256) {
        const int n = (int)(i % N);
        const size_t m = i / N;
        float v = ws[i];
        for (int z = 1; z < splits; ++z) v += ws[(size_t)z * total + i];
        v += bias[n];
        if (relu) v = fmaxf(v, 0.f);
        y[m * ldy + n] = v;
    }
}

__global__ __launch_bounds__(256)
void softmax_rows_kernel(const float* __restrict__ x, int ldx, float* __restrict__ y, int M, int ncls)
{
    const int row = blockIdx.x * 4 + (threadIdx.x >> 6);
    const int lane = threadIdx.x & 63;
    if (row >= M) return;
    const float* xr = x + (size_t)row * ldx;
    const float v0 = lane < ncls ? xr[lane] : -INFINITY, v1 = lane + 64 < ncls ? xr[lane + 64] : -INFINITY;
    float mx = fmaxf(v0, v1);
#pragma unroll
    for (int o = 32; o > 0; o >>= 1) mx = fmaxf(mx, __shfl_xor(mx, o));
    const float e0 = lane < ncls ? expf(v0 - mx) : 0.f, e1 = lane + 64 < ncls ? expf(v1 - mx) : 0.f;
    double sum = (double)e0 + (double)e1;
#pragma unroll
    for (int o = 32; o > 0; o >>= 1) sum += __shfl_xor(sum, o);
    if (lane < ncls) y[(size_t)row * ncls + lane] = (float)((double)e0 / sum);
    if (lane + 64 < ncls) y[(size_t)row * ncls + lane + 64] = (float)((double)e1 / sum);
}

__global__ __launch_bounds__(256)
void head_finish_kernel(const float* __restrict__ x, int ldx, int M, int ncls, int ndelta,
                        float* __restrict__ classes, float* __restrict__ deltas)
{
    const int row = blockIdx.x * 4 + (threadIdx.x >> 6);
    const int lane = threadIdx.x & 63;
    if (row >= M) return;
    const float* xr = x + (size_t)row * ldx;
    const float v0 = lane < ncls ? xr[lane] : -INFINITY, v1 = lane + 64 < ncls ? xr[lane + 64] : -INFINITY;
    float mx = fmaxf(v0, v1);
#pragma unroll
    for (int o = 32; o > 0; o >>= 1) mx = fmaxf(mx, __shfl_xor(mx, o));
    const float e0 = lane < ncls ? expf(v0 - mx) : 0.f, e1 = lane + 64 < ncls ? expf(v1 - mx) : 0.f;
    float sum = e0 + e1;
#pragma unroll
    for (int o = 32; o > 0; o >>= 1) sum += __shfl_xor(sum, o);
    if (lane < ncls) classes[(size_t)row * ncls + lane] = e0 / sum;
    if (lane + 64 < ncls) classes[(size_t)row * ncls + lane + 64] = e1 / sum;
    for (int j = lane; j < ndelta; j += 64) deltas[(size_t)row * ndelta + j] = xr[ncls + j];
}

__global__ void pack_fc_chw_to_hwc_kernel(const float* __restrict__ w, float* __restrict__ wp,
                                          int out_f, int c, int hw)
{
    const size_t K = (size_t)c * hw;
    const size_t total = (size_t)out_f * K;
    for (size_t i = (size_t)blockIdx.x * 256 + threadIdx.x; i < total; i += (size_t)gridDim.x * 256) {
        const size_t o = i / K, kk = i % K;
        const int p = (int)(kk / c), ch = (int)(kk % c);
        wp[i] = w[o * K + (size_t)ch * hw + p];
    }
}

__global__ void pack_stack_rows_kernel(const float* __restrict__ w1, const float* __restrict__ b1, int n1,
                                       const float* __restrict__ w2, const float* __restrict__ b2, int n2,
                                       int k, int n_pad, float* __restrict__ wo, float* __restrict__ bo)
{
    const size_t total = (size_t)n_pad * k;
    for (size_t i = (size_t)blockIdx.x * 256 + threadIdx.x; i < total; i += (size_t)gridDim.x * 256) {
        const int row = (int)(i / k), col = (int)(i % k);
        float v = 0.f;
        if (row < n1) v = w1[(size_t)row * k + col];
        else if (row < n1 + n2) v = w2[(size_t)(row - n1) * k + col];
        wo[i] = v;
        if (col == 0) bo[row] = row < n1 ? b1[row] : (row < n1 + n2 ? b2[row - n1] : 0.f);
    }
}

struct LinearPlan { bool big; int mblocks, nblocks, splits, stages_per_split; };

static LinearPlan plan_linear(int M, int N, int K)
{
    LinearPlan p;
    p.big = (M <= 320) || (M % 320 == 0);
    const int bm = p.big ? 320 : 128;
    p.mblocks = cdiv(M, bm);
    p.nblocks = cdiv(N, 128);
    const int stages = K / 16;
    static int target = -1;
    if (target < 0) { const char* e = frcnn_knob("FRCNN_LINEAR_BLOCKS_TARGET"); target = e ? atoi(e) : 256; if (target < 1) target = 1; }
    int want = target / (p.mblocks * p.nblocks);
    int cap = stages / 8;
    if (cap < 1) cap = 1;
    if (want > cap) want = cap;
    if (want < 1) want = 1;
    p.stages_per_split = cdiv(stages, want);
    p.splits = cdiv(stages, p.stages_per_split);
    return p;
}

size_t linear_workspace_bytes(int M, int N, int K)
{
    if (M < 1 || N < 1 || K < 16) return 0;
    const LinearPlan p = plan_linear(M, N, K);
    return p.splits > 1 ? (size_t)p.splits * M * N * sizeof(float) : 0;
}

template <int TM, int TN, int WM, int WN>
static int launch_linear_cfg(const LinearPlan& p, const float* a, int lda, const float* w,
                             const float* bias, float* y, int ldy, float* ws, int M, int N, int K,
                             int relu, hipStream_t s)
{
    using C = GemmCfg<TM, TN, WM, WN>;
    auto kern = linear_mfma_kernel<TM, TN, WM, WN, false>;
    FRCNN_MAX_LDS_ONCE(kern, C::LDS_BYTES);
    dim3 grid(p.nblocks, p.mblocks, p.splits);
    hipLaunchKernelGGL(kern, grid, dim3(C::THREADS), C::LDS_BYTES, s, a, lda, w, bias, y, ldy, ws, M, N, K,
                       p.stages_per_split, relu, BatchGeom{0, 0, 0, 0, 0, 0});
    return check_launch();
}

template <int TM, int TN, int WM, int WN, int NSETS>
static int launch_linear_batched_cfg(const float* a, int lda, const float* w, float* y, int ldy, int M, int N, int K,
                                     const BatchGeom& bg, hipStream_t s)
{
    using C = GemmCfg<TM, TN, WM, WN>;
    auto kern = linear_mfma_kernel<TM, TN, WM, WN, true, NSETS>;
    FRCNN_MAX_LDS_ONCE(kern, C::LDS_BYTES);
    const long long total = (long long)bg.nblocks * bg.mblocks * bg.batches;
    if (total < 1 || total > 0x7fffffffLL) return FRCNN_EINVAL;
    hipLaunchKernelGGL(kern, dim3((unsigned)total), dim3(C::THREADS), C::LDS_BYTES, s, a, lda, w,
                       (const float*)nullptr, y, ldy, (float*)nullptr, M, N, K, K >> 4, 0, bg);
    return check_launch();
}

static thread_local int g_batched_tile = 0;
void linear_batched_set_tile(int rows) { g_batched_tile = rows; }

int launch_linear_batched(const float* a, int lda, size_t a_stride, const float* w, size_t w_stride, float* y, int ldy,
                          size_t y_stride, int M, int N, int K, int batches, hipStream_t s)
{
    if (M < 1 || N < 1 || K < 16 || K % 16 != 0 || lda % 4 != 0 || lda < K || ldy < N || batches < 1) return FRCNN_EINVAL;
    static int env_tile = -1;
    if (env_tile < 0) { const char* e = frcnn_knob("FRCNN_WINO_TILE"); env_tile = e ? atoi(e) : 0; }
    const int tile = env_tile ? env_tile : (g_batched_tile ? g_batched_tile : 64);
    BatchGeom bg{(long long)a_stride, (long long)w_stride, (long long)y_stride, cdiv(N, 128), cdiv(M, 128), batches};
    if (tile == 128) return launch_linear_batched_cfg<2, 2, 2, 2, 1>(a, lda, w, y, ldy, M, N, K, bg, s);
    bg.mblocks = cdiv(M, 64);
    return launch_linear_batched_cfg<1, 2, 2, 2, 1>(a, lda, w, y, ldy, M, N, K, bg, s);
}

int launch_linear(const float* a, int lda, const float* w, const float* bias, float* y, int ldy,
                  int M, int N, int K, unsigned flags, void* ws, size_t ws_bytes, hipStream_t s)
{
    if (M < 1 || N < 1 || K < 16 || K % 16 != 0 || lda % 4 != 0 || lda < K || ldy < N) return FRCNN_EINVAL;
    const LinearPlan p = plan_linear(M, N, K);
    const size_t need = p.splits > 1 ? (size_t)p.splits * M * N * sizeof(float) : 0;
    if (need > ws_bytes || (need > 0 && ws == nullptr)) return FRCNN_EINVAL;
    const int relu = (flags & FRCNN_RELU) ? 1 : 0;
    int rc = p.big ? launch_linear_cfg<5, 1, 2, 4>(p, a, lda, w, bias, y, ldy, (float*)ws, M, N, K, relu, s)
                   : launch_linear_cfg<2, 2, 2, 2>(p, a, lda, w, bias, y, ldy, (float*)ws, M, N, K, relu, s);
    if (rc != FRCNN_OK) return rc;
    if (p.splits > 1) {
        const size_t total = (size_t)M * N;
        int blocks = (int)((total + 255) / 256);
        if (blocks > 2048) blocks = 2048;
        hipLaunchKernelGGL(splitk_reduce_kernel, dim3(blocks), dim3(256), 0, s, (const float*)ws, bias,
                           y, ldy, M, N, p.splits, relu);
        rc = check_launch();
    }
    return rc;
}

int launch_softmax_rows(const float* x, int ldx, float* y, int M, int ncls, hipStream_t s)
{
    if (M < 1 || ncls < 1 || ncls > 128 || ldx < ncls) return FRCNN_EINVAL;
    hipLaunchKernelGGL(softmax_rows_kernel, dim3(cdiv(M, 4)), dim3(256), 0, s, x, ldx, y, M, ncls);
    return check_launch();
}

int launch_head_finish(const float* x, int ldx, int M, int ncls, int ndelta, float* classes,
                       float* deltas, hipStream_t s)
{
    if (M < 1 || ncls < 1 || ncls > 128 || ndelta < 0 || ldx < ncls + ndelta) return FRCNN_EINVAL;
    hipLaunchKernelGGL(head_finish_kernel, dim3(cdiv(M, 4)), dim3(256), 0, s, x, ldx, M, ncls, ndelta,
                       classes, deltas);
    return check_launch();
}

int launch_pack_fc_chw_to_hwc(const float* w, float* wp, int out_f, int c, int phw, hipStream_t s)
{
    if (out_f < 1 || c < 1 || phw < 1) return FRCNN_EINVAL;
    hipLaunchKernelGGL(pack_fc_chw_to_hwc_kernel, dim3(8192), dim3(256), 0, s, w, wp, out_f, c, phw);
    return check_launch();
}

int launch_pack_stack_rows(const float* w1, const float* b1, int n1, const float* w2, const float* b2,
                           int n2, int k, int n_pad, float* wo, float* bo, hipStream_t s)
{
    if (n1 < 0 || n2 < 0 || n1 + n2 > n_pad || k < 1) return FRCNN_EINVAL;
    const size_t total = (size_t)n_pad * k;
    int blocks = (int)((total + 255) / 256);
    if (blocks > 2048) blocks = 2048;
    hipLaunchKernelGGL(pack_stack_rows_kernel, dim3(blocks), dim3(256), 0, s, w1, b1, n1, w2, b2, n2, k,
                       n_pad, wo, bo);
    return check_launch();
}

}
```

fasterrcnn_amd/csrc/proposals.hip:

```cpp
#include "geometry.h"
#include <type_traits>

namespace frcnn {

typedef unsigned long long u64;

__device__ __forceinline__ unsigned ordered_bits(float f)
{
    const unsigned b = __float_as_uint(f);
    return (b & 0x80000000u) ? ~b : (b | 0x80000000u);
}
__device__ __forceinline__ float from_ordered_bits(unsigned o)
{
    const unsigned b = (o & 0x80000000u) ? (o & 0x7fffffffu) : ~o;
    return __uint_as_float(b);
}

__global__ __launch_bounds__(256)
void rpn_decode_kernel(const float* __restrict__ head, int ld, const float* __restrict__ anchors,
                       const float* __restrict__ valid, int A, float* __restrict__ scores,
                       f32x4* __restrict__ boxes_all, u64* __restrict__ keys)
{
    const int n = blockIdx.x * 256 + threadIdx.x;
    if (n >= A) return;
    const int pix = n / 9, k = n - pix * 9;
    const float* row = head + (size_t)pix * ld;
    const float logit = row[k];
    const float score = 1.0f / (1.0f + expf(-logit));
    const float dy = row[9 + 4 * k + 0], dx = row[9 + 4 * k + 1];
    const float dh = row[9 + 4 * k + 2], dw = row[9 + 4 * k + 3];
    const f32x4 a = reinterpret_cast<const f32x4*>(anchors)[n];
    const float cy = __fadd_rn(__fmul_rn(a[2], dy), a[0]);
    const float cx = __fadd_rn(__fmul_rn(a[3], dx), a[1]);
    const float h = __fmul_rn(a[2], expf(dh));
    const float w = __fmul_rn(a[3], expf(dw));
    const float hh = 0.5f * h, hw = 0.5f * w;
    f32x4 b;
    b[0] = cy - hh; b[1] = cx - hw; b[2] = cy + hh; b[3] = cx + hw;
    scores[n] = score;
    boxes_all[n] = b;
    const bool ok = (valid == nullptr) || (valid[n] > 0.f);
    keys[n] = ok ? (((u64)ordered_bits(score) << 32) | (u64)(unsigned)(n + 1)) : 0ull;
}

__global__ __launch_bounds__(256)
void nms_keys_kernel(const float* __restrict__ scores, int n, u64* __restrict__ keys)
{
    const int i = blockIdx.x * 256 + threadIdx.x;
    if (i >= n) return;
    const float f = scores[i];
    const unsigned hi = f != f ? 0u : ordered_bits(f == 0.f ? 0.f : f);
    keys[i] = ((u64)hi << 32) | (u64)(0xFFFFFFFFu - (unsigned)i);
}

__device__ __forceinline__ u64 shfl_xor_u64(u64 v, int lane_mask)
{
    const unsigned lo = __shfl_xor((unsigned)(v & 0xFFFFFFFFull), lane_mask);
    const unsigned hi = __shfl_xor((unsigned)(v >> 32), lane_mask);
    return ((u64)hi << 32) | lo;
}

__device__ __forceinline__ u64 bitonic_pick(u64 mine, u64 other, int g, int j, int k)
{
    const bool keep_max = (((g & k) == 0) == ((g & j) == 0));
    const bool other_bigger = other > mine;
    return (keep_max == other_bigger) ? other : mine;
}

template <int PER, int J>
__device__ __forceinline__ void bitonic_inthread(u64 (&e)[PER], int base, int k)
{
#pragma unroll
    for (int r = 0; r < PER; ++r) {
        if ((r & J) == 0) {
            const u64 a = e[r], b = e[r | J];
            e[r] = bitonic_pick(a, b, base + r, J, k);
            e[r | J] = bitonic_pick(b, a, base + (r | J), J, k);
        }
    }
}

template <int PER>
__device__ void bitonic_sort_regs(u64* buf, int tid)
{
    constexpr int N = 1024 * PER;
    u64 e[PER];
    const int base = tid * PER;
#pragma unroll
    for (int r = 0; r < PER; ++r) e[r] = buf[base + r];
    for (int k = 2; k <= N; k <<= 1) {
        for (int j = k >> 1; j > 0; j >>= 1) {
            if (j >= 64 * PER) {
#pragma unroll
                for (int r = 0; r < PER; ++r) buf[base + r] = e[r];
                __syncthreads();
#pragma unroll
                for (int r = 0; r < PER; ++r) e[r] = bitonic_pick(e[r], buf[(base + r) ^ j], base + r, j, k);
                __syncthreads();
            } else if (j >= PER) {
                const int lane_mask = j / PER;
#pragma unroll
                for (int r = 0; r < PER; ++r) e[r] = bitonic_pick(e[r], shfl_xor_u64(e[r], lane_mask), base + r, j, k);
            } else {
                if (PER > 8 && j == 8) bitonic_inthread<PER, (PER > 8 ? 8 : 1)>(e, base, k);
                else if (PER > 4 && j == 4) bitonic_inthread<PER, (PER > 4 ? 4 : 1)>(e, base, k);
                else if (PER > 2 && j == 2) bitonic_inthread<PER, (PER > 2 ? 2 : 1)>(e, base, k);
                else if (PER > 1 && j == 1) bitonic_inthread<PER, 1>(e, base, k);
            }
        }
    }
#pragma unroll
    for (int r = 0; r < PER; ++r) buf[base + r] = e[r];
    __syncthreads();
// ... 244 lines not shown
        }
        int incl = local;
        for (int o = 1; o < 64; o <<= 1) {
            const int v = __shfl_up(incl, o);
            if ((tid & 63) >= o) incl += v;
        }
        if ((tid & 63) == 63) wave_tot[tid >> 6] = incl;
        __syncthreads();
        int wave_off = 0;
        for (int wv = 0; wv < (tid >> 6); ++wv) wave_off += wave_tot[wv];
        pos = wave_off + incl - local;
        for (int q = 0; q < per; ++q) {
            const int p = tid * per + q;
            if (p < want && p < sort_n) {
                const u64 k = buf[p];
                const unsigned low = (unsigned)(k & 0xFFFFFFFFull);
                const int idx = MODE == 0 ? (int)(low - 1u) : (int)(0xFFFFFFFFu - low);
                f32x4 b = boxes_src[idx];
                bool keep = true;
                if (MODE == 0) {
                    b[0] = fmaxf(b[0], 0.f); b[1] = fmaxf(b[1], 0.f);
                    b[2] = fminf(b[2], image_h); b[3] = fminf(b[3], image_w);
                    keep = ((b[2] - b[0]) >= min_side) && ((b[3] - b[1]) >= min_side);
                }
                if (keep) {
                    cand_boxes[pos] = b;
                    cand_scores[pos] = from_ordered_bits((unsigned)(k >> 32));
                    ++pos;
                }
            }
        }
    }
    if (tid == 1023) { counts[0] = want; counts[1] = pos; }
#ifdef TOPK_CLOCKS
    tk[5] = __builtin_readcyclecounter();
    if (tid == 0 && n_keys > 20000) printf("topk cycles: load %llu  select %llu  gather %llu  sort %llu  emit %llu\n", tk[1] - tk[0], tk[2] - tk[1], tk[3] - tk[2], tk[4] - tk[3], tk[5] - tk[4]);
#endif
}

__global__ __launch_bounds__(1024)
void topk_rank_kernel(const u64* __restrict__ sel, const int32_t* __restrict__ counts, int sort_n, const f32x4* __restrict__ boxes_src,
                      float image_h, float image_w, float min_side, int32_t* __restrict__ sorted_idx, f32x4* __restrict__ tmp_boxes,
                      float* __restrict__ tmp_scores, int32_t* __restrict__ keep_flag)
{
    extern __shared__ __attribute__((aligned(16))) unsigned char smem_rank[];
    u64* lk = reinterpret_cast<u64*>(smem_rank);
    int* part = reinterpret_cast<int*>(lk + sort_n);
    const int n = counts[0];
    const int k0 = blockIdx.x * 32;
    if (k0 >= n) return;
    const int tid = threadIdx.x;
    const int npad = (n + 31) & ~31;
    for (int i = tid; i < npad; i += 1024) lk[i] = i < n ? sel[i] : 0ull;
    __syncthreads();
    const int kb = tid & 31, seg = tid >> 5;
    const int seg_len = npad >> 5;
    const u64 mine = k0 + kb < n ? lk[k0 + kb] : ~0ull;
    const u64* p = lk + seg * seg_len;
    int cnt = 0;
    int j = 0;
    for (; j + 4 <= seg_len; j += 4) {
        const u64 a = p[j], b = p[j + 1], c = p[j + 2], d = p[j + 3];
        cnt += (a > mine) + (b > mine) + (c > mine) + (d > mine);
    }
    for (; j < seg_len; ++j) cnt += p[j] > mine;
    part[kb * 32 + seg] = cnt;
    __syncthreads();
    if (tid < 32 && k0 + tid < n) {
        int rank = 0;
#pragma unroll
        for (int q = 0; q < 32; ++q) rank += part[tid * 32 + ((q + tid) & 31)];
        const u64 k = lk[k0 + tid];
        const int idx = (int)((unsigned)(k & 0xFFFFFFFFull) - 1u);
        f32x4 b = boxes_src[idx];
        b[0] = fmaxf(b[0], 0.f); b[1] = fmaxf(b[1], 0.f);
        b[2] = fminf(b[2], image_h); b[3] = fminf(b[3], image_w);
        if (sorted_idx) sorted_idx[rank] = idx;
        tmp_boxes[rank] = b;
        tmp_scores[rank] = from_ordered_bits((unsigned)(k >> 32));
        keep_flag[rank] = (((b[2] - b[0]) >= min_side) && ((b[3] - b[1]) >= min_side)) ? 1 : 0;
    }
}

__global__ __launch_bounds__(1024)
void topk_emit_kernel(const f32x4* __restrict__ tmp_boxes, const float* __restrict__ tmp_scores, const int32_t* __restrict__ keep_flag,
                      int sort_n, f32x4* __restrict__ cand_boxes, float* __restrict__ cand_scores, int32_t* __restrict__ counts)
{
    __shared__ int wave_tot[16];
    const int tid = threadIdx.x;
    const int n = counts[0];
    auto body = [&](auto perc) {
        constexpr int PER = decltype(perc)::value;
        int fl[PER];
        f32x4 bx[PER];
        float sc[PER];
#pragma unroll
        for (int q = 0; q < PER; ++q) {
            const int r = tid * PER + q;
            const bool in = r < n;
            fl[q] = in ? keep_flag[r] : 0;
            bx[q] = in ? tmp_boxes[r] : f32x4{0.f, 0.f, 0.f, 0.f};
            sc[q] = in ? tmp_scores[r] : 0.f;
        }
        int local = 0;
#pragma unroll
        for (int q = 0; q < PER; ++q) local += fl[q] ? 1 : 0;
        int incl = local;
        for (int o = 1; o < 64; o <<= 1) {
            const int v = __shfl_up(incl, o);
            if ((tid & 63) >= o) incl += v;
        }
        if ((tid & 63) == 63) wave_tot[tid >> 6] = incl;
        __syncthreads();
        int wave_off = 0;
        for (int wv = 0; wv < (tid >> 6); ++wv) wave_off += wave_tot[wv];
        int pos = wave_off + incl - local;
#pragma unroll
        for (int q = 0; q < PER; ++q) {
            if (fl[q]) {
                cand_boxes[pos] = bx[q];
                cand_scores[pos] = sc[q];
                ++pos;
            }
        }
        if (tid == 1023) counts[1] = pos;
    };
    const int per = sort_n >> 10 ? sort_n >> 10 : 1;
    if (per == 8) body(std::integral_constant<int, 8>());
    else if (per == 16) body(std::integral_constant<int, 16>());
    else if (per == 4) body(std::integral_constant<int, 4>());
    else if (per == 2) body(std::integral_constant<int, 2>());
    else body(std::integral_constant<int, 1>());
}

static constexpr int NMS_BAND = 32;

__host__ __device__ __forceinline__ int nms_tri(int k) { return k * (k + 1) / 2; }

__global__ __launch_bounds__(64)
void nms_mask_kernel(const f32x4* __restrict__ boxes, const int32_t* __restrict__ n_ptr, float thr,
                     int nw_stride, u64* __restrict__ mask, int bx_begin, const int32_t* __restrict__ done)
{
    if (done != nullptr && *done != 0) return;
    const int n = *n_ptr;
    const int tile = nms_tri(bx_begin) + (int)blockIdx.x;
    int bx = (int)((sqrtf(8.f * (float)tile + 1.f) - 1.f) * 0.5f);
    while (nms_tri(bx + 1) <= tile) ++bx;
    while (nms_tri(bx) > tile) --bx;
    const int by = tile - nms_tri(bx);
    if (bx * 64 >= n) return;
    __shared__ f32x4 colb[64];
    const int t = threadIdx.x;
    const int jn = bx * 64 + t;
    colb[t] = jn < n ? boxes[jn] : f32x4{0.f, 0.f, 0.f, 0.f};
    __syncthreads();
    const int i = by * 64 + t;
    if (i >= n) return;
    const f32x4 a = boxes[i];
    u64 bits = 0ull;
    const int jmax = (n - bx * 64) < 64 ? (n - bx * 64) : 64;
    for (int j = 0; j < jmax; ++j) {
        const int jj = bx * 64 + j;
        if (jj > i && iou_gt(a, colb[j], thr)) bits |= 1ull << j;
    }
    mask[(size_t)i * nw_stride + bx] = bits;
}

__device__ __forceinline__ u64 readlane64(u64 v, int lane_uniform)
{
    const int l = __builtin_amdgcn_readfirstlane(lane_uniform);
    const unsigned lo = (unsigned)__builtin_amdgcn_readlane((int)(unsigned)(v & 0xFFFFFFFFull), l);
    const unsigned hi = (unsigned)__builtin_amdgcn_readlane((int)(unsigned)(v >> 32), l);
    return ((u64)hi << 32) | lo;
}

static constexpr int NMS_PIECES = 24;
static constexpr int NMS_DMA = 1 + NMS_PIECES;
static constexpr int NMS_SLOT_BYTES = NMS_DMA * 1024;
static constexpr int NMS_LDS_BYTES = 2 * NMS_SLOT_BYTES;
typedef __attribute__((address_space(3))) void* nms_lds_ptr;
static_assert(NMS_DMA <= 63, "the look-ahead must fit the 6-bit vmcnt");

#ifdef NMS_CLOCKS
#define NMS_T(k) do { const unsigned long long _t = __builtin_amdgcn_s_memrealtime(); if ((k) != 0 || nms_tl != 0) nms_acc[k] += (float)(_t - nms_tl); nms_tl = _t; } while (0)
#else
#define NMS_T(k) do { } while (0)
#endif

__global__ __launch_bounds__(64)
void nms_reduce_kernel(const u64* __restrict__ mask, int nw_stride, const int32_t* __restrict__ n_ptr,
                       int max_keep, const f32x4* __restrict__ cand_boxes,
                       const int32_t* __restrict__ order,
                       int32_t* __restrict__ keep, f32x4* __restrict__ props,
                       int32_t* __restrict__ n_keep_out,
                       int c_limit,
                       const int32_t* __restrict__ done_in,
                       int32_t* __restrict__ done_out)
{
    if (done_in != nullptr && *done_in != 0) return;
    extern __shared__ __attribute__((aligned(16))) unsigned char nms_ring_lds[];
    unsigned char* const ring = nms_ring_lds;
    __shared__ int32_t kept_list[2048];
    __shared__ u64 kb_list[256];
    const int n = *n_ptr;
    const int lane = threadIdx.x;
    const int nw = (n + 63) >> 6;
    const bool wide = nw > 128;
    u64 rem[4] = {0ull, 0ull, 0ull, 0ull};
#ifdef NMS_CLOCKS
    float nms_acc[8] = {0, 0, 0, 0, 0, 0, 0, 0};
    unsigned long long nms_tl = 0;
    const unsigned long long nms_t_in = __builtin_amdgcn_s_memrealtime();
#endif
    int room = max_keep;
    int c_done = 0;
    u64 fq = 0ull;
    const int wl0 = min(2 * lane, nw_stride - 2), wl1 = min(128 + 2 * lane, nw_stride - 2);

    const __amdgpu_buffer_rsrc_t mrs = __builtin_amdgcn_make_buffer_rsrc(const_cast<u64*>(mask), 0, 0x7fffffff, 0x00020000);
    auto dma16 = [&](const u64* g, unsigned char* l) {
        __builtin_amdgcn_raw_ptr_buffer_load_lds(mrs, (nms_lds_ptr)l, 16, (int)((const unsigned char*)g - (const unsigned char*)mask), 0, 0, 0);
    };
    const int row_bytes = nw_stride * 8, vo0 = wl0 * 8, vo1 = wl1 * 8;
    auto dma_piece = [&](int row_index, bool upper, unsigned char* l) {
        __builtin_amdgcn_raw_ptr_buffer_load_lds(mrs, (nms_lds_ptr)l, 16, upper ? vo1 : vo0, row_index * row_bytes, 0, 0);
    };
    auto issue_band = [&](int c, unsigned char* slot) {
        const int row = min(c * 64 + lane, n - 1);
        dma16(mask + (size_t)row * nw_stride + min(c, nw_stride - 1), slot);
    };
    auto or16 = [&](const uint4& v, int q0) {
        rem[q0] |= ((u64)v.y << 32) | v.x;
        rem[q0 + 1] |= ((u64)v.w << 32) | v.z;
    };

    if (n > 0) {
        for (int p = 0; p < 2; ++p) {
            unsigned char* slot = ring + p * NMS_SLOT_BYTES;
            issue_band(p, slot);
#pragma unroll
            for (int u = 0; u < NMS_PIECES; ++u) dma_piece(0, wide && (u & 1), slot + 1024 + u * 1024);
        }
        const int c_end = min(nw, c_limit);
        for (int c = 0; c < c_end; ++c) {
            NMS_T(0);
            unsigned char* slot = ring + (c & 1) * NMS_SLOT_BYTES;
            const unsigned la = (unsigned)(size_t)slot + 16u * (unsigned)lane;
            uint4 bnd, r0[NMS_PIECES];
// ... 127 lines not shown
                kept_list[before++] = c * 64 + b;
            }
        }
        kept = total;
    }
    __syncthreads();
    for (int k = lane; k < max_keep; k += 64) {
        if (k < kept) {
            const int ci = kept_list[k];
            if (keep) keep[k] = order ? order[ci] : ci;
            if (props) props[k] = cand_boxes[ci];
        } else {
            if (props) props[k] = f32x4{0.f, 0.f, 0.f, 0.f};
        }
    }
    if (lane == 0) *n_keep_out = kept;
#ifdef NMS_CLOCKS
    if (lane == 0 && props && max_keep >= 4) {
        const unsigned long long t_out = __builtin_amdgcn_s_memrealtime();
        props[max_keep - 1] = f32x4{nms_acc[1], nms_acc[2], nms_acc[3], nms_acc[4]};
        props[max_keep - 2] = f32x4{nms_acc[5], nms_acc[6], (float)(t_out - nms_t_in), (float)c_done};
        props[max_keep - 3] = f32x4{nms_acc[0], nms_acc[7], (float)n, (float)kept};
        props[max_keep - 4] = f32x4{done_in != nullptr ? 1.f : 0.f, (float)c_limit, 0.f, 0.f};
    }
#endif
}
#undef NMS_T

static size_t align_up(size_t v, size_t a) { return (v + a - 1) / a * a; }

size_t proposal_scratch_bytes(int a_cap, int pre_cap, int post_cap)
{
    size_t b = 0;
    b += align_up((size_t)a_cap * 8, 256);
    b += align_up((size_t)a_cap * 16, 256);
    b += align_up((size_t)pre_cap * 16, 256);
    b += align_up((size_t)pre_cap * 4, 256);
    b += align_up((size_t)pre_cap * (pre_cap / 64) * 8 + 256, 256);
    b += align_up((size_t)post_cap * 4, 256);
    return b;
}

void proposal_scratch_carve(ProposalScratch& ps, void* base, int a_cap, int pre_cap, int post_cap)
{
    unsigned char* p = static_cast<unsigned char*>(base);
    ps.keys = reinterpret_cast<u64*>(p);         p += align_up((size_t)a_cap * 8, 256);
    ps.boxes_all = reinterpret_cast<float*>(p);  p += align_up((size_t)a_cap * 16, 256);
    ps.cand_boxes = reinterpret_cast<float*>(p); p += align_up((size_t)pre_cap * 16, 256);
    ps.cand_scores = reinterpret_cast<float*>(p); p += align_up((size_t)pre_cap * 4, 256);
    ps.mask = reinterpret_cast<u64*>(p);         p += align_up((size_t)pre_cap * (pre_cap / 64) * 8 + 256, 256);
    ps.keep = reinterpret_cast<int32_t*>(p);
    ps.a_cap = a_cap; ps.pre_cap = pre_cap; ps.post_cap = post_cap;
}

static int pow2_at_least(int v) { int p = 1024; while (p < v) p <<= 1; return p; }

template <int MODE>
static int launch_topk(const u64* keys, int n_keys, int K, const float* boxes_src, float ih, float iw,
                       float min_side, int32_t* sorted_idx, float* cand_boxes, float* cand_scores,
                       int32_t* counts, hipStream_t s, void* tmp = nullptr)
{
    const int sort_n = pow2_at_least(K);
    if (sort_n > 16384) return FRCNN_EUNSUPPORTED;
    const size_t lds = (size_t)sort_n * 8 + 4096 * 4 + 64 * 4;
    static const bool no_split = frcnn_knob("FRCNN_TOPK_ONE_BLOCK") != nullptr;
    if (MODE == 0 && tmp != nullptr && !no_split) {
        unsigned char* tb = static_cast<unsigned char*>(tmp);
        u64* sel = reinterpret_cast<u64*>(tb);
        f32x4* tboxes = reinterpret_cast<f32x4*>(tb + (size_t)sort_n * 8);
        float* tscores = reinterpret_cast<float*>(tb + (size_t)sort_n * 24);
        int32_t* flags = reinterpret_cast<int32_t*>(tb + (size_t)sort_n * 28);
        auto k1 = topk_sort_kernel<0, true>;
        FRCNN_MAX_LDS_ONCE(k1, 16384 * 8 + 4096 * 4 + 64 * 4);
        hipLaunchKernelGGL(k1, dim3(1), dim3(1024), lds, s, keys, n_keys, K, sort_n, reinterpret_cast<const f32x4*>(boxes_src), ih, iw,
                           min_side, sorted_idx, reinterpret_cast<f32x4*>(cand_boxes), cand_scores, counts, sel);
        int rc = check_launch();
        if (rc) return rc;
        const size_t lds2 = (size_t)sort_n * 8 + 32 * 32 * 4;
        FRCNN_MAX_LDS_ONCE(topk_rank_kernel, 16384 * 8 + 32 * 32 * 4);
        hipLaunchKernelGGL(topk_rank_kernel, dim3(cdiv(K, 32)), dim3(1024), lds2, s, sel, counts, sort_n,
                           reinterpret_cast<const f32x4*>(boxes_src), ih, iw, min_side, sorted_idx, tboxes, tscores, flags);
        rc = check_launch();
        if (rc) return rc;
        hipLaunchKernelGGL(topk_emit_kernel, dim3(1), dim3(1024), 0, s, tboxes, tscores, flags, sort_n, reinterpret_cast<f32x4*>(cand_boxes),
                           cand_scores, counts);
        return check_launch();
    }
    auto kern = topk_sort_kernel<MODE>;
    FRCNN_MAX_LDS_ONCE(kern, 16384 * 8 + 4096 * 4 + 64 * 4);
    hipLaunchKernelGGL(kern, dim3(1), dim3(1024), lds, s, keys, n_keys, K, sort_n,
                       reinterpret_cast<const f32x4*>(boxes_src), ih, iw, min_side, sorted_idx,
                       reinterpret_cast<f32x4*>(cand_boxes), cand_scores, counts, (u64*)nullptr);
    return check_launch();
}

static int launch_nms_phases(const ProposalScratch& ps, const int32_t* n_ptr, int nw, bool banded, float thr, int max_keep,
                             const int32_t* order, int32_t* keep, f32x4* props, int32_t* n_keep, hipStream_t s)
{
    const int nw_stride = ps.pre_cap / 64;
    const f32x4* boxes = reinterpret_cast<const f32x4*>(ps.cand_boxes);
    int32_t* done = ps.keep;
    FRCNN_MAX_LDS_ONCE(nms_reduce_kernel, NMS_LDS_BYTES);
    int rc;
    if (!banded) {
        hipLaunchKernelGGL(nms_mask_kernel, dim3(nms_tri(nw)), dim3(64), 0, s, boxes, n_ptr, thr, nw_stride, ps.mask, 0, (const int32_t*)nullptr);
        rc = check_launch();
        if (rc) return rc;
        hipLaunchKernelGGL(nms_reduce_kernel, dim3(1), dim3(64), NMS_LDS_BYTES, s, ps.mask, nw_stride, n_ptr, max_keep, boxes, order, keep,
                           props, n_keep, nw, (const int32_t*)nullptr, (int32_t*)nullptr);
        return check_launch();
    }
    hipLaunchKernelGGL(nms_mask_kernel, dim3(nms_tri(NMS_BAND)), dim3(64), 0, s, boxes, n_ptr, thr, nw_stride, ps.mask, 0, (const int32_t*)nullptr);
    rc = check_launch();
    if (rc) return rc;
    hipLaunchKernelGGL(nms_reduce_kernel, dim3(1), dim3(64), NMS_LDS_BYTES, s, ps.mask, nw_stride, n_ptr, max_keep, boxes, order, keep,
                       props, n_keep, NMS_BAND, (const int32_t*)nullptr, done);
    rc = check_launch();
    if (rc) return rc;
    hipLaunchKernelGGL(nms_mask_kernel, dim3(nms_tri(nw) - nms_tri(NMS_BAND)), dim3(64), 0, s, boxes, n_ptr, thr, nw_stride, ps.mask, NMS_BAND,
                       (const int32_t*)done);
    rc = check_launch();
    if (rc) return rc;
    hipLaunchKernelGGL(nms_reduce_kernel, dim3(1), dim3(64), NMS_LDS_BYTES, s, ps.mask, nw_stride, n_ptr, max_keep, boxes, order, keep,
                       props, n_keep, nw, (const int32_t*)done, done);
    return check_launch();
}

int launch_rpn_proposals(const ProposalScratch& ps, const float* head, int ld_head,
                         const float* anchor_map, const float* valid_map, int fh, int fw,
                         int image_h, int image_w, int pre_nms, int post_nms, float nms_thr,
                         float min_side, float* scores, int32_t* sorted_idx, float* props,
                         int32_t* counts, hipStream_t s)
{
    const int A = fh * fw * 9;
    if (A < 1 || A > ps.a_cap || pre_nms < 1 || pre_nms > ps.pre_cap || post_nms < 1 ||
        post_nms > ps.post_cap || post_nms > 2048 || ld_head < 45)
        return FRCNN_EINVAL;
    hipLaunchKernelGGL(rpn_decode_kernel, dim3(cdiv(A, 256)), dim3(256), 0, s, head, ld_head, anchor_map,
                       valid_map, A, scores, reinterpret_cast<f32x4*>(ps.boxes_all), ps.keys);
    int rc = check_launch();
    if (rc) return rc;
    rc = launch_topk<0>(ps.keys, A, pre_nms, ps.boxes_all, (float)image_h, (float)image_w, min_side,
                        sorted_idx, ps.cand_boxes, ps.cand_scores, counts, s, ps.mask);
    if (rc) return rc;
    return launch_nms_phases(ps, counts + 1, cdiv(pre_nms, 64), cdiv(pre_nms, 64) > NMS_BAND, nms_thr, post_nms, nullptr, nullptr,
                             reinterpret_cast<f32x4*>(props), counts + 2, s);
}

int launch_nms(const ProposalScratch& ps, const float* boxes, const float* scores, int n, float thr,
               int max_keep, int32_t* keep, int32_t* n_keep, hipStream_t s)
{
    if (n < 0 || n > ps.pre_cap || n > ps.a_cap || max_keep < 1 || max_keep > 2048) return FRCNN_EINVAL;
    if (n == 0) {
        FRCNN_HIP_TRY(hipMemsetAsync(n_keep, 0, sizeof(int32_t), s));
        return FRCNN_OK;
    }
    hipLaunchKernelGGL(nms_keys_kernel, dim3(cdiv(n, 256)), dim3(256), 0, s, scores, n, ps.keys);
    int rc = check_launch();
    if (rc) return rc;
    int32_t* order = reinterpret_cast<int32_t*>(ps.boxes_all);
    int32_t* counts = order + ps.a_cap;
    rc = launch_topk<1>(ps.keys, n, n, boxes, 0.f, 0.f, 0.f, order, ps.cand_boxes, ps.cand_scores, counts, s);
    if (rc) return rc;
    const int nw = cdiv(n, 64);
    const bool banded = nw >= 2 * NMS_BAND && 4 * max_keep <= 64 * NMS_BAND;
    return launch_nms_phases(ps, counts + 1, nw, banded, thr, max_keep, order, keep, nullptr, n_keep, s);
}

}
```

include/frcnn_hip.h:

```cpp
#ifndef FRCNN_HIP_H
#define FRCNN_HIP_H

#include <stddef.h>
#include <stdint.h>

#ifdef __cplusplus
extern "C" {
#endif

#define FRCNN_OK            0
#define FRCNN_EINVAL       -1
#define FRCNN_EHIP         -2
#define FRCNN_ENOMEM       -3
#define FRCNN_EUNSUPPORTED -4
#define FRCNN_ENODEVICE    -5

#define FRCNN_ABI_VERSION 21

#define FRCNN_RELU   1u
#define FRCNN_POOL2  2u
#define FRCNN_X3G_WSPLIT 0x800u

int         frcnn_abi_version(void);
const char* frcnn_error_string(int code);
const char* frcnn_last_hip_error(void);
int         frcnn_device_count(void);

int frcnn_anchors(int image_h, int image_w, int fh, int fw, int feature_pixels,
                  float* d_anchor_map, float* d_valid_map, void* stream);

size_t frcnn_preprocess_workspace_bytes(int H, int W, int out_h, int out_w);
int frcnn_preprocess(const unsigned char* d_rgb, int H, int W, int out_h, int out_w, int bgr_order,
                     int horizontal_flip, float scaling, const float* means, const float* stds,
                     float* d_out, unsigned char* d_out_u8, void* d_ws, size_t ws_bytes, void* stream);

int frcnn_rpn_targets(const float* d_anchor_map, const float* d_valid_map, int n_anchors,
                      const float* d_gt_boxes, int n_gt, double object_thr, double background_thr,
                      float* d_rpn_map, int32_t* d_object_idx, int32_t* d_background_idx, int32_t* d_counts,
                      void* d_ws, void* stream);

int frcnn_pack_conv3x3(const float* d_w_oihw, float* d_w_packed, int cout, int cin, void* stream);
int frcnn_pack_conv3x3_c3(const float* d_w_oihw, float* d_w_packed, int cout, void* stream);
int frcnn_pack_fc_chw_to_hwc(const float* d_w, float* d_w_packed, int out_features, int channels,
                             int pooled_hw, void* stream);
int frcnn_pack_stack_rows(const float* d_w1, const float* d_b1, int n1,
                          const float* d_w2, const float* d_b2, int n2,
                          int k, int n_pad, float* d_w_out, float* d_b_out, void* stream);

int frcnn_conv3x3_c3(const float* d_x_chw, const float* d_w_packed, const float* d_bias,
                     float* d_y, int H, int W, int cout, unsigned flags, void* stream);
int frcnn_conv3x3_c3_cmax(const float* d_x_chw, const float* d_w_packed, const float* d_bias,
                          float* d_y, int H, int W, int cout, unsigned flags, float* d_cmax_out, void* stream);
size_t frcnn_conv3x3_workspace_bytes(int H, int W, int cin, int cout);
int frcnn_conv3x3_nhwc(const float* d_x, const float* d_w_packed, const float* d_bias,
                       float* d_y, int H, int W, int cin, int cout, unsigned flags,
                       void* d_ws, size_t ws_bytes, void* stream);
int frcnn_conv3x3_uses_winograd(int cin, int cout);
int frcnn_resnet_block_uses_winograd(int width, int stride);
int frcnn_pack_conv3x3_winograd(const float* d_w_oihw, const float* d_row_scale, float* d_u, int cout, int cin, void* stream);
int frcnn_pack_conv3x3_winograd_taps(const float* d_w_packed, float* d_u, int cout, int cin, int data_gradient, void* stream);
size_t frcnn_conv3x3_winograd_workspace_bytes(int n_maps, int H, int W, int cin, int cout);
int frcnn_conv3x3_nhwc_winograd(const float* d_x, const float* d_u, const float* d_bias,
                                float* d_y, int n_maps, int H, int W, int cin, int cout, unsigned flags,
                                void* d_ws, size_t ws_bytes, void* stream);
int frcnn_conv3x3_uses_winograd_fused(int cin, int cout);
int frcnn_resnet_block_uses_winograd_fused(int n_maps, int width, int stride);
int frcnn_pack_conv3x3_winograd_fused(const float* d_w_oihw, const float* d_row_scale, float* d_u, int cout, int cin, void* stream);
int frcnn_pack_conv3x3_winograd_fused_taps(const float* d_w_packed, float* d_u, int cout, int cin, int data_gradient, void* stream);
int frcnn_conv3x3_nhwc_winograd_fused(const float* d_x, const float* d_u, const float* d_bias, float* d_y,
                                      int H, int W, int cin, int cout, unsigned flags, void* stream);
int frcnn_conv3x3_nhwc_winograd_fused_maps(const float* d_x, const float* d_u, const float* d_bias, float* d_y, int n_maps,
                                           int H, int W, int cin, int cout, unsigned flags, void* stream);

#define FRCNN_X6T_ROW_TILE 320
#define FRCNN_X6T_COL_TILE 256
size_t frcnn_x6t_record_bytes(int rows_padded, int K);
int frcnn_split_rows_x6t(const float* d_a, int lda, size_t a_batch_floats, void* d_rec, int rows, int rows_padded, int K, int batches,
                         void* stream);
size_t frcnn_gemm_x6t_workspace_bytes(int M, int N, int K, int batches);
int frcnn_gemm_x6t(const void* d_a_rec, int a_rows, size_t a_batch_bytes, const void* d_b_rec, int b_rows, size_t b_batch_bytes,
                   const float* d_bias, const float* d_residual, float* d_c, int ldc, size_t c_batch_floats, int M, int N, int K,
                   int batches, unsigned flags, void* d_ws, size_t ws_bytes, void* stream);
int frcnn_pixel_absmax(const float* d_x, float* d_cmax, long long pixels, int c, void* stream);
int frcnn_split_pixels_x3t(const float* d_x, const float* d_cmax, void* d_rec, float* d_inv_scale, int n_maps, int H, int W, int c, int stride,
                           int rows_padded, void* stream);
int frcnn_split_patches3x3_x3t(const float* d_x, const float* d_cmax, void* d_rec, float* d_inv_scale, int n_maps, int H, int W, int c,
                               int stride, int rows_padded, void* stream);
size_t frcnn_x3t_blob_bytes(int rows_padded, int K, int batches);
int frcnn_pack_rows_x3t(const float* d_a, int lda, size_t a_batch_floats, void* d_blob, int rows, int rows_padded, int K, int batches,
                        void* stream);
size_t frcnn_conv3x3_winograd_x3_pack_bytes(int cout, int cin);
int frcnn_pack_conv3x3_winograd_x3(const float* d_u_f32, void* d_blob, int cout, int cin, void* stream);
size_t frcnn_conv3x3_winograd_x3_workspace_bytes(int n_maps, int H, int W, int cin, int cout);
int frcnn_conv3x3_nhwc_winograd_x3(const float* d_x, const void* d_blob, const float* d_bias, float* d_y, int n_maps, int H, int W, int cin,
                                   int cout, unsigned flags, void* d_ws, size_t ws_bytes, void* stream);
size_t frcnn_conv3x3_winograd_x3_fused_workspace_bytes(int n_maps, int H, int W);
int frcnn_conv3x3_nhwc_winograd_x3_fused(const float* d_x, const void* d_blob, const float* d_bias, float* d_y, int n_maps, int H, int W,
                                         int cin, int cout, unsigned flags, void* d_ws, size_t ws_bytes, void* stream);
int frcnn_conv3x3_nhwc_winograd_x3_chain(const float* d_x, const void* d_blob, const float* d_bias, float* d_y, int n_maps, int H, int W, int cin,
                                         int cout, unsigned flags, int one_launch, void* d_ws, size_t ws_bytes, const float* d_cmax_in,
                                         float* d_cmax_out, void* stream);
size_t frcnn_x3t_record_bytes(int rows_padded, int K);
int frcnn_rows_scale_x3t(const float* d_a, int lda, size_t a_batch_floats, float* d_inv_scale, int rows, int rows_padded, int K, int batches,
                         void* stream);
int frcnn_split_rows_x3t(const float* d_a, int lda, size_t a_batch_floats, const float* d_inv_scale, void* d_rec, int rows, int rows_padded,
                         int K, int batches, void* stream);
size_t frcnn_gemm_x3t_workspace_bytes(int M, int N, int K, int batches);
int frcnn_gemm_x3t(const void* d_a_rec, const float* d_a_inv, int a_rows, size_t a_batch_bytes, size_t a_inv_batch_floats,
                   const void* d_b_rec, const float* d_b_inv, int b_rows, size_t b_batch_bytes, size_t b_inv_batch_floats,
                   const float* d_bias, const float* d_residual, float* d_c, int ldc, size_t c_batch_floats, int M, int N, int K,
                   int batches, unsigned flags, void* d_ws, size_t ws_bytes, void* stream);

int frcnn_split_pixels_x6t(const float* d_x, void* d_rec, int N, int H, int W, int C, int stride, int rows_padded, void* stream);
int frcnn_conv3x3_uses_winograd_x6(int cin, int cout);
size_t frcnn_conv3x3_winograd_x6_pack_bytes(int cout, int cin);
int frcnn_pack_conv3x3_winograd_x6(const float* d_w_oihw, const float* d_row_scale, void* d_u_rec, int cout, int cin, void* stream);
size_t frcnn_conv3x3_winograd_x6_workspace_bytes(int n_maps, int H, int W, int cin, int cout);
int frcnn_conv3x3_nhwc_winograd_x6(const float* d_x, const void* d_u_rec, const float* d_bias, float* d_y, int n_maps, int H, int W, int cin,
                                   int cout, unsigned flags, void* d_ws, size_t ws_bytes, void* stream);
int frcnn_split_patches3x3_x6t(const float* d_x, void* d_rec, int N, int H, int W, int C, int stride, int rows_padded, void* stream);
int frcnn_maxpool2x2_nhwc(const float* d_x, float* d_y, int H, int W, int c, void* stream);

int frcnn_fold_bn_pack(const float* d_w_oihw, const float* d_gamma, const float* d_beta,
                       const float* d_mean, const float* d_var, float eps, int cout, int cin, int ksize,
                       float* d_w_packed, float* d_b_packed, void* stream);
size_t frcnn_conv_workspace_bytes(int N, int H, int W, int cin, int cout, int ksize, int stride, int pad);
int frcnn_conv_nhwc(const float* d_x, const float* d_w_packed, const float* d_bias, const float* d_residual,
                    float* d_y, int N, int H, int W, int cin, int cout, int ksize, int stride, int pad,
                    unsigned flags, void* d_ws, size_t ws_bytes, void* stream);
int frcnn_conv7x7_s2_c3(const float* d_x_chw, const float* d_w_packed, const float* d_bias, float* d_y,
                        int H, int W, int cout, unsigned flags, void* stream);
int frcnn_maxpool3x3_s2_nhwc(const float* d_x, float* d_y, int H, int W, int c, void* stream);
int frcnn_spatial_mean_nhwc(const float* d_x, float* d_y, int N, int H, int W, int c, void* stream);

size_t frcnn_linear_workspace_bytes(int M, int N, int K);
int frcnn_linear(const float* d_a, int lda, const float* d_w, const float* d_bias,
                 float* d_y, int ldy, int M, int N, int K, unsigned flags,
                 void* d_ws, size_t ws_bytes, void* stream);
int frcnn_softmax_rows(const float* d_x, int ldx, float* d_y, int M, int ncls, void* stream);

typedef struct frcnn_ctx frcnn_ctx;

int frcnn_rpn_proposals(frcnn_ctx* ctx, const float* d_head, int ld_head,
                        const float* d_anchor_map, const float* d_valid_map,
                        int fh, int fw, int image_h, int image_w,
                        int pre_nms, int post_nms, float nms_threshold, float min_side,
                        float* d_scores, int32_t* d_sorted_idx, float* d_props, int32_t* d_counts,
                        void* stream);

int frcnn_nms(frcnn_ctx* ctx, const float* d_boxes, const float* d_scores, int n, float threshold,
              int max_keep, int32_t* d_keep, int32_t* d_n_keep, void* stream);

int frcnn_roi_pool(const float* d_fm, int fh, int fw, int c, const float* d_rois,
                   const int32_t* d_n_rois, int max_rois, int pooled, float spatial_scale,
                   float* d_out, void* stream);
int frcnn_roi_pool_x3t(const float* d_fm, int fh, int fw, int c, const float* d_rois, const int32_t* d_n_rois, int max_rois, int pooled,
                       float spatial_scale, float* d_cmax, float* d_inv_scale, void* d_rec, int rec_rows, void* stream);
int frcnn_roi_align(const float* d_fm, int fh, int fw, int c, const float* d_rois, const int32_t* d_n_rois, int max_rois,
                    int pooled, float spatial_scale, int sampling_ratio, int aligned, float* d_out, void* stream);
int frcnn_roi_align_backward(const float* d_rois, int n_rois, int fh, int fw, int c, int pooled, float spatial_scale,
                             int sampling_ratio, int aligned, const float* d_dout, float* d_dfm, int accumulate, void* stream);

int frcnn_ops_roi_align(const float* d_x, int n_img, int fh, int fw, int c, const float* d_rois, int k, int out_h, int out_w,
                        float spatial_scale, int sampling_ratio, int aligned, float* d_out, void* stream);
int frcnn_ops_roi_align_backward(const float* d_rois, int k, int n_img, int fh, int fw, int c, int out_h, int out_w, float spatial_scale,
                                 int sampling_ratio, int aligned, const float* d_dout, float* d_dx, void* stream);
int frcnn_ops_ms_roi_align(const float* const* d_x, const int* fh, const int* fw, const float* scales, int n_levels, int n_img, int c,
                           const float* d_rois, int k, int out_h, int out_w, int sampling_ratio, float canonical_scale,
                           float canonical_level, int k_min, int k_max, float* d_out, void* stream);
size_t frcnn_ops_ms_roi_align_workspace_bytes(int k, int n_levels, int n_img);
int frcnn_ops_ms_roi_align_backward(const float* d_rois, int k, const int* fh, const int* fw, const float* scales, int n_levels, int n_img,
                                    int c, int out_h, int out_w, int sampling_ratio, float canonical_scale, float canonical_level,
                                    int k_min, int k_max, const float* d_dout, float* const* d_dx, void* d_ws, size_t ws_bytes,
                                    void* stream);
int frcnn_ops_roi_pool(const float* d_x, int n_img, int fh, int fw, int c, const float* d_rois, int k, int out_h, int out_w,
                       float spatial_scale, float* d_out, int32_t* d_argmax, void* stream);
int frcnn_ops_roi_pool_backward(const float* d_rois, int k, int n_img, int fh, int fw, int c, int out_h, int out_w, float spatial_scale,
                                const int32_t* d_argmax, const float* d_dout, float* d_dx, void* stream);
size_t frcnn_ops_nms_workspace_bytes(int n);
int frcnn_ops_nms(const void* d_boxes, int boxes_f64, const int64_t* d_order, const int64_t* d_categories, int n, float iou_threshold,
                  uint8_t* d_keep, void* d_ws, size_t ws_bytes, void* stream);

#define FRCNN_OPS_F16  1
#define FRCNN_OPS_BF16 2
int frcnn_ops_half_run(void);
int frcnn_ops_roi_align_16(int elem_type, const void* d_x, int n_img, int fh, int fw, int c, const float* d_rois, int k, int out_h,
                           int out_w, float spatial_scale, int sampling_ratio, int aligned, void* d_out, void* stream);
int frcnn_ops_roi_align_backward_16(int elem_type, const float* d_rois, int k, int n_img, int fh, int fw, int c, int out_h, int out_w,
                                    float spatial_scale, int sampling_ratio, int aligned, const void* d_dout, void* d_dx, void* stream);
int frcnn_ops_roi_pool_16(int elem_type, const void* d_x, int n_img, int fh, int fw, int c, const float* d_rois, int k, int out_h,
                          int out_w, float spatial_scale, void* d_out, int32_t* d_argmax, void* stream);
int frcnn_ops_roi_pool_backward_16(int elem_type, const float* d_rois, int k, int n_img, int fh, int fw, int c, int out_h, int out_w,
                                   float spatial_scale, const int32_t* d_argmax, const void* d_dout, void* d_dx, void* stream);
int frcnn_ops_ms_roi_align_16(int elem_type, const void* const* d_x, const int* fh, const int* fw, const float* scales, int n_levels,
                              int n_img, int c, const float* d_rois, int k, int out_h, int out_w, int sampling_ratio,
                              float canonical_scale, float canonical_level, int k_min, int k_max, void* d_out, void* stream);
int frcnn_ops_ms_roi_align_backward_16(int elem_type, const float* d_rois, int k, const int* fh, const int* fw, const float* scales,
                                       int n_levels, int n_img, int c, int out_h, int out_w, int sampling_ratio, float canonical_scale,
                                       float canonical_level, int k_min, int k_max, const void* d_dout, void* const* d_dx, void* d_ws,
                                       size_t ws_bytes, void* stream);

int frcnn_ops_ps_roi_pool(const float* d_x, int n_img, int fh, int fw, int c, const float* d_rois, int k, int out_h, int out_w,
                          float spatial_scale, float* d_out, void* stream);
int frcnn_ops_ps_roi_pool_backward(const float* d_rois, int k, int n_img, int fh, int fw, int c, int out_h, int out_w, float spatial_scale,
                                   const float* d_dout, float* d_dx, void* stream);
int frcnn_ops_ps_roi_align(const float* d_x, int n_img, int fh, int fw, int c, const float* d_rois, int k, int out_h, int out_w,
                           float spatial_scale, int sampling_ratio, float* d_out, void* stream);
int frcnn_ops_ps_roi_align_backward(const float* d_rois, int k, int n_img, int fh, int fw, int c, int out_h, int out_w, float spatial_scale,
                                    int sampling_ratio, const float* d_dout, float* d_dx, void* stream);
int frcnn_ops_ps_roi_pool_16(int elem_type, const void* d_x, int n_img, int fh, int fw, int c, const float* d_rois, int k, int out_h,
                             int out_w, float spatial_scale, void* d_out, void* stream);
int frcnn_ops_ps_roi_pool_backward_16(int elem_type, const float* d_rois, int k, int n_img, int fh, int fw, int c, int out_h, int out_w,
                                      float spatial_scale, const void* d_dout, void* d_dx, void* stream);
int frcnn_ops_ps_roi_align_16(int elem_type, const void* d_x, int n_img, int fh, int fw, int c, const float* d_rois, int k, int out_h,
                              int out_w, float spatial_scale, int sampling_ratio, void* d_out, void* stream);
int frcnn_ops_ps_roi_align_backward_16(int elem_type, const float* d_rois, int k, int n_img, int fh, int fw, int c, int out_h, int out_w,
                                       float spatial_scale, int sampling_ratio, const void* d_dout, void* d_dx, void* stream);

typedef struct frcnn_deform_geom {
    int32_t c_in, height, width, c_out, kernel_h, kernel_w, stride_h, stride_w, pad_h, pad_w, dilation_h, dilation_w, groups,
            offset_groups;
// ... 469 lines not shown
```

Before: 984.9.

## Fuse split-K reduce into RPN decode and head softmax; add small linear tiles

The split-K partial-plane reduction for the RPN head GEMM now happens inside the proposal decode kernel, and for the detector head it is folded into a combined reduce+softmax+delta-split kernel. This removes separate reduce and finish launches plus a memset. Linear planning gains smaller 64x64 and 64x128 tiles for narrow or short GEMMs. NMS mask tiles are split across 4 waves, and top-k emission is spread over multiple blocks. Together these cut launch overhead and idle compute units in the small tail stages, at the cost of more template variants and extra redundant plane reads.

```diff
diff --git a/fasterrcnn_amd/_native.py b/fasterrcnn_amd/_native.py
--- a/fasterrcnn_amd/_native.py
+++ b/fasterrcnn_amd/_native.py
@@ -10,6 +10,7 @@
           -4: "FRCNN_EUNSUPPORTED", -5: "FRCNN_ENODEVICE"}
 RELU = 1
 POOL2 = 2
+LINEAR_WHOLE_TILES = 0x100
 NUM_KCLASS = 11
 KCLASS_NAMES = ("conv3x3_mfma", "conv3x3_c3", "linear_mfma", "proposals", "roi_pool", "other", "winograd_transforms",
                 "winograd_gemm", "winograd_x6_transforms", "winograd_x6_gemm", "winograd_x3f")
@@ -19,7 +20,7 @@
     "frcnn_anchors", "frcnn_pack_conv3x3", "frcnn_pack_conv3x3_c3", "frcnn_pack_fc_chw_to_hwc",
     "frcnn_pack_stack_rows", "frcnn_conv3x3_c3", "frcnn_conv3x3_c3_cmax", "frcnn_conv3x3_workspace_bytes", "frcnn_conv3x3_nhwc",
     "frcnn_maxpool2x2_nhwc",
-    "frcnn_linear_workspace_bytes", "frcnn_linear", "frcnn_softmax_rows", "frcnn_rpn_proposals",
+    "frcnn_linear_workspace_bytes", "frcnn_linear", "frcnn_linear_heads", "frcnn_softmax_rows", "frcnn_rpn_proposals",
     "frcnn_nms", "frcnn_roi_pool", "frcnn_roi_pool_x3t", "frcnn_detections", "frcnn_ctx_create", "frcnn_ctx_create_proposals", "frcnn_ctx_destroy",
     "frcnn_ctx_bytes", "frcnn_vgg16_forward", "frcnn_ctx_tensor", "frcnn_ctx_timing_enable",
     "frcnn_ctx_timing_read",
@@ -376,6 +377,7 @@
     "frcnn_conv3x3_nhwc_winograd_fused": (C.c_int, [_vp, _vp, _vp, _vp, _i, _i, _i, _i, _u, _vp]),
     "frcnn_linear_workspace_bytes": (C.c_size_t, [_i, _i, _i]),
     "frcnn_linear": (C.c_int, [_vp, _i, _vp, _vp, _vp, _i, _i, _i, _i, _u, _vp, _sz, _vp]),
+    "frcnn_linear_heads": (C.c_int, [_vp, _i, _vp, _vp, _vp, _i, _i, _i, _i, _i, _u, _vp, _sz, _vp, _vp, _vp]),
     "frcnn_softmax_rows": (C.c_int, [_vp, _i, _vp, _i, _i, _vp]),
     "frcnn_rpn_proposals": (C.c_int, [_vp, _vp, _i, _vp, _vp, _i, _i, _i, _i, _i, _i, _f, _f,
                                       _vp, _vp, _vp, _vp, _vp]),
diff --git a/fasterrcnn_amd/csrc/api.hip b/fasterrcnn_amd/csrc/api.hip
--- a/fasterrcnn_amd/csrc/api.hip
+++ b/fasterrcnn_amd/csrc/api.hip
@@ -573,6 +573,14 @@
     return launch_linear(d_a, lda, d_w, d_bias, d_y, ldy, M, N, K, flags, d_ws, ws_bytes, as_stream(stream));
 }
 
+int frcnn_linear_heads(const float* d_a, int lda, const float* d_w, const float* d_bias, float* d_logits, int ld, int M, int ncls,
+                       int ndelta, int K, unsigned flags, void* d_ws, size_t ws_bytes, float* d_classes, float* d_deltas, void* stream)
+{
+    if (!d_a || !d_w || !d_bias || !d_logits || !d_classes || !d_deltas || (flags & ~FRCNN_LINEAR_WHOLE_TILES)) return FRCNN_EINVAL;
+    return launch_linear_heads(d_a, lda, d_w, d_bias, d_logits, ld, M, ncls, ndelta, K, flags, d_ws, ws_bytes, d_classes, d_deltas,
+                               as_stream(stream));
+}
+
 int frcnn_softmax_rows(const float* d_x, int ldx, float* d_y, int M, int ncls, void* stream)
 {
     if (!d_x || !d_y) return FRCNN_EINVAL;
@@ -1231,7 +1239,9 @@
                         int C, const float* d_anchor_map, const float* d_valid_map, float* d_props, int32_t* d_counts, hipStream_t s)
 {
     int rc;
-    STEP(2, launch_linear(c->rpn_trunk, C, head_w, head_b, c->rpn_head, 128, fh * fw, 45, C, 0u, c->lin_ws, c->lin_ws_bytes, s));
+    int splits = 1;
+    STEP(2, launch_linear_planes(c->rpn_trunk, C, head_w, head_b, c->rpn_head, 128, fh * fw, 45, C, 0u, c->lin_ws, c->lin_ws_bytes, &splits, s));
+    const HeadPlanes planes{static_cast<const float*>(c->lin_ws), head_b, c->rpn_head, splits};
     const float* amap = d_anchor_map;
     const float* vmap = d_valid_map;
     if (!amap || !vmap) {
@@ -1241,10 +1251,9 @@
         }
         amap = c->anchor_map; vmap = c->valid_map;
     }
-    FRCNN_HIP_TRY(hipMemsetAsync(d_counts, 0, 4 * sizeof(int32_t), s));
     STEP(3, launch_rpn_proposals(c->ps, c->rpn_head, 128, amap, p->allow_edge_proposals ? nullptr : vmap, fh, fw,
                                  H, W, p->pre_nms, p->post_nms, p->rpn_nms_threshold, p->min_side, c->scores,
-                                 c->sorted_idx, d_props, d_counts, s));
+                                 c->sorted_idx, d_props, d_counts, s, splits > 1 ? &planes : nullptr));
     return FRCNN_OK;
 }
 
@@ -1264,8 +1273,8 @@
     const int nd = (ncls - 1) * 4;
     const int hld = cdiv(ncls + nd, 128) * 128;
     c->last_head_ld = hld;
-    STEP(2, launch_linear(c->fc2_out, V, head_w, head_b, c->head_logits, hld, n_rois, ncls + nd, V, 0u, c->lin_ws, c->lin_ws_bytes, s));
-    STEP(5, launch_head_finish(c->head_logits, hld, n_rois, ncls, nd, d_classes, d_deltas, s));
+    STEP(2, launch_linear_heads(c->fc2_out, V, head_w, head_b, c->head_logits, hld, n_rois, ncls, nd, V, 0u, c->lin_ws, c->lin_ws_bytes,
+                                d_classes, d_deltas, s));
     return FRCNN_OK;
 }
 }
diff --git a/fasterrcnn_amd/csrc/common.h b/fasterrcnn_amd/csrc/common.h
--- a/fasterrcnn_amd/csrc/common.h
+++ b/fasterrcnn_amd/csrc/common.h
@@ -102,6 +102,10 @@
 size_t linear_workspace_bytes(int M, int N, int K);
 int launch_linear(const float* a, int lda, const float* w, const float* bias, float* y, int ldy,
                   int M, int N, int K, unsigned flags, void* ws, size_t ws_bytes, hipStream_t s);
+int launch_linear_planes(const float* a, int lda, const float* w, const float* bias, float* y, int ldy, int M, int N, int K, unsigned flags,
+                         void* ws, size_t ws_bytes, int* splits, hipStream_t s);
+int launch_linear_heads(const float* a, int lda, const float* w, const float* bias, float* logits, int ld, int M, int ncls, int ndelta,
+                        int K, unsigned flags, void* ws, size_t ws_bytes, float* classes, float* deltas, hipStream_t s);
 int launch_linear_batched(const float* a, int lda, size_t a_stride, const float* w, size_t w_stride, float* y, int ldy,
                           size_t y_stride, int M, int N, int K, int batches, hipStream_t s);
 void linear_batched_set_tile(int rows);
@@ -201,11 +205,12 @@
 size_t proposal_scratch_bytes(int a_cap, int pre_cap, int post_cap);
 void   proposal_scratch_carve(ProposalScratch& ps, void* base, int a_cap, int pre_cap, int post_cap);
 
+struct HeadPlanes { const float* ws; const float* bias; float* head_out; int splits; };
 int launch_rpn_proposals(const ProposalScratch& ps, const float* head, int ld_head,
                          const float* anchor_map, const float* valid_map, int fh, int fw,
                          int image_h, int image_w, int pre_nms, int post_nms, float nms_thr,
                          float min_side, float* scores, int32_t* sorted_idx, float* props,
-                         int32_t* counts, hipStream_t s);
+                         int32_t* counts, hipStream_t s, const HeadPlanes* planes = nullptr);
 int launch_nms(const ProposalScratch& ps, const float* boxes, const float* scores, int n, float thr,
                int max_keep, int32_t* keep, int32_t* n_keep, hipStream_t s);
 
diff --git a/fasterrcnn_amd/csrc/linear.hip b/fasterrcnn_amd/csrc/linear.hip
--- a/fasterrcnn_amd/csrc/linear.hip
+++ b/fasterrcnn_amd/csrc/linear.hip
@@ -256,6 +256,40 @@
     for (int j = lane; j < ndelta; j += 64) deltas[(size_t)row * ndelta + j] = xr[ncls + j];
 }
 
+__global__ __launch_bounds__(64)
+void heads_reduce_finish_kernel(const float* __restrict__ ws, const float* __restrict__ bias, float* __restrict__ logits, int ld, int M,
+                                int ncls, int ndelta, int splits, float* __restrict__ classes, float* __restrict__ deltas)
+{
+    const int row = blockIdx.x, lane = threadIdx.x;
+    const int N = ncls + ndelta;
+    const size_t plane = (size_t)M * N;
+    const float* const wr = ws + (size_t)row * N;
+    float v0 = -INFINITY, v1 = -INFINITY;
+    for (int n = lane; n < N; n += 64) {
+        float v = wr[n];
+        for (int z0 = 1; z0 < splits; z0 += 16) {
+            float t[16];
+#pragma unroll
+            for (int q = 0; q < 16; ++q) t[q] = z0 + q < splits ? wr[(size_t)(z0 + q) * plane + n] : 0.f;
+#pragma unroll
+            for (int q = 0; q < 16; ++q) if (z0 + q < splits) v += t[q];
+        }
+        v += bias[n];
+        logits[(size_t)row * ld + n] = v;
+        if (n < ncls) { if (n < 64) v0 = v; else v1 = v; }
+        else deltas[(size_t)row * ndelta + (n - ncls)] = v;
+    }
+    float mx = fmaxf(v0, v1);
+#pragma unroll
+    for (int o = 32; o > 0; o >>= 1) mx = fmaxf(mx, __shfl_xor(mx, o));
+    const float e0 = lane < ncls ? expf(v0 - mx) : 0.f, e1 = lane + 64 < ncls ? expf(v1 - mx) : 0.f;
+    float sum = e0 + e1;
+#pragma unroll
+    for (int o = 32; o > 0; o >>= 1) sum += __shfl_xor(sum, o);
+    if (lane < ncls) classes[(size_t)row * ncls + lane] = e0 / sum;
+    if (lane + 64 < ncls) classes[(size_t)row * ncls + lane + 64] = e1 / sum;
+}
+
 __global__ void pack_fc_chw_to_hwc_kernel(const float* __restrict__ w, float* __restrict__ wp,
                                           int out_f, int c, int hw)
 {
@@ -283,13 +317,15 @@
     }
 }
 
-struct LinearPlan { bool big; int mblocks, nblocks, splits, stages_per_split; };
-
-static LinearPlan plan_linear(int M, int N, int K)
+enum LinearTile { TILE_320x128 = 0, TILE_128x128 = 1, TILE_64x128 = 2, TILE_64x64 = 3 };
+struct LinearPlan { int tile; int mblocks, nblocks, splits, stages_per_split; };
+
+static LinearPlan plan_linear(int M, int N, int K, bool whole_tiles = false)
 {
     LinearPlan p;
-    p.big = (M <= 320) || (M % 320 == 0);
-    const int bm = p.big ? 320 : 128;
+    const bool big = (M <= 320) || (M % 320 == 0);
+    const int bm = big ? 320 : 128;
+    p.tile = big ? TILE_320x128 : TILE_128x128;
     p.mblocks = cdiv(M, bm);
     p.nblocks = cdiv(N, 128);
     const int stages = K / 16;
@@ -302,6 +338,11 @@
     if (want < 1) want = 1;
     p.stages_per_split = cdiv(stages, want);
     p.splits = cdiv(stages, p.stages_per_split);
+    static const bool knob_whole = frcnn_knob("FRCNN_LINEAR_WHOLE_TILES") != nullptr;
+    if (!whole_tiles && !knob_whole) {
+        if (N <= 64) { p.tile = TILE_64x64; p.mblocks = cdiv(M, 64); p.nblocks = 1; }
+        else if (M <= 320 && N < 1024) { p.tile = TILE_64x128; p.mblocks = cdiv(M, 64); }
+    }
     return p;
 }
 
@@ -356,26 +397,64 @@
     return launch_linear_batched_cfg<1, 2, 2, 2, 1>(a, lda, w, y, ldy, M, N, K, bg, s);
 }
 
+static int launch_linear_gemm(const LinearPlan& p, const float* a, int lda, const float* w, const float* bias, float* y, int ldy, float* ws,
+                              int M, int N, int K, int relu, hipStream_t s)
+{
+    switch (p.tile) {
+    case TILE_320x128: return launch_linear_cfg<5, 1, 2, 4>(p, a, lda, w, bias, y, ldy, ws, M, N, K, relu, s);
+    case TILE_128x128: return launch_linear_cfg<2, 2, 2, 2>(p, a, lda, w, bias, y, ldy, ws, M, N, K, relu, s);
+    case TILE_64x128:  return launch_linear_cfg<1, 1, 2, 4>(p, a, lda, w, bias, y, ldy, ws, M, N, K, relu, s);
+    case TILE_64x64:   return launch_linear_cfg<1, 1, 2, 2>(p, a, lda, w, bias, y, ldy, ws, M, N, K, relu, s);
+    }
+    return FRCNN_EINVAL;
+}
+
 int launch_linear(const float* a, int lda, const float* w, const float* bias, float* y, int ldy,
                   int M, int N, int K, unsigned flags, void* ws, size_t ws_bytes, hipStream_t s)
 {
-    if (M < 1 || N < 1 || K < 16 || K % 16 != 0 || lda % 4 != 0 || lda < K || ldy < N) return FRCNN_EINVAL;
-    const LinearPlan p = plan_linear(M, N, K);
-    const size_t need = p.splits > 1 ? (size_t)p.splits * M * N * sizeof(float) : 0;
-    if (need > ws_bytes || (need > 0 && ws == nullptr)) return FRCNN_EINVAL;
-    const int relu = (flags & FRCNN_RELU) ? 1 : 0;
-    int rc = p.big ? launch_linear_cfg<5, 1, 2, 4>(p, a, lda, w, bias, y, ldy, (float*)ws, M, N, K, relu, s)
-                   : launch_linear_cfg<2, 2, 2, 2>(p, a, lda, w, bias, y, ldy, (float*)ws, M, N, K, relu, s);
+    int splits = 1;
+    int rc = launch_linear_planes(a, lda, w, bias, y, ldy, M, N, K, flags, ws, ws_bytes, &splits, s);
     if (rc != FRCNN_OK) return rc;
-    if (p.splits > 1) {
+    if (splits > 1) {
         const size_t total = (size_t)M * N;
         int blocks = (int)((total + 255) / 256);
         if (blocks > 2048) blocks = 2048;
         hipLaunchKernelGGL(splitk_reduce_kernel, dim3(blocks), dim3(256), 0, s, (const float*)ws, bias,
-                           y, ldy, M, N, p.splits, relu);
+                           y, ldy, M, N, splits, (flags & FRCNN_RELU) ? 1 : 0);
         rc = check_launch();
     }
     return rc;
+}
+
+int launch_linear_planes(const float* a, int lda, const float* w, const float* bias, float* y, int ldy, int M, int N, int K, unsigned flags,
+                         void* ws, size_t ws_bytes, int* splits, hipStream_t s)
+{
+    if (M < 1 || N < 1 || K < 16 || K % 16 != 0 || lda % 4 != 0 || lda < K || ldy < N) return FRCNN_EINVAL;
+    const LinearPlan p = plan_linear(M, N, K, (flags & FRCNN_LINEAR_WHOLE_TILES) != 0);
+    const size_t need = p.splits > 1 ? (size_t)p.splits * M * N * sizeof(float) : 0;
+    if (need > ws_bytes || (need > 0 && ws == nullptr)) return FRCNN_EINVAL;
+    *splits = p.splits;
+    return launch_linear_gemm(p, a, lda, w, bias, y, ldy, (float*)ws, M, N, K, (flags & FRCNN_RELU) ? 1 : 0, s);
+}
+
+int launch_linear_heads(const float* a, int lda, const float* w, const float* bias, float* logits, int ld, int M, int ncls, int ndelta,
+                        int K, unsigned flags, void* ws, size_t ws_bytes, float* classes, float* deltas, hipStream_t s)
+{
+    if (ncls < 1 || ncls > 128 || ndelta < 0) return FRCNN_EINVAL;
+    const int N = ncls + ndelta;
+    if (M < 1 || K < 16 || K % 16 != 0 || lda % 4 != 0 || lda < K || ld < N) return FRCNN_EINVAL;
+    static const bool knob_unfused = frcnn_knob("FRCNN_HEADS_UNFUSED") != nullptr;
+    if ((flags & FRCNN_LINEAR_WHOLE_TILES) != 0 || knob_unfused) {
+        const int rc = launch_linear(a, lda, w, bias, logits, ld, M, N, K, flags & FRCNN_LINEAR_WHOLE_TILES, ws, ws_bytes, s);
+        return rc != FRCNN_OK ? rc : launch_head_finish(logits, ld, M, ncls, ndelta, classes, deltas, s);
+    }
+    int splits = 1;
+    const int rc = launch_linear_planes(a, lda, w, bias, logits, ld, M, N, K, 0u, ws, ws_bytes, &splits, s);
+    if (rc != FRCNN_OK) return rc;
+    if (splits == 1) return launch_head_finish(logits, ld, M, ncls, ndelta, classes, deltas, s);
+    hipLaunchKernelGGL(heads_reduce_finish_kernel, dim3(M), dim3(64), 0, s, (const float*)ws, bias, logits, ld, M, ncls, ndelta, splits,
+                       classes, deltas);
+    return check_launch();
 }
 
 int launch_softmax_rows(const float* x, int ldx, float* y, int M, int ncls, hipStream_t s)
diff --git a/fasterrcnn_amd/csrc/proposals.hip b/fasterrcnn_amd/csrc/proposals.hip
--- a/fasterrcnn_amd/csrc/proposals.hip
+++ b/fasterrcnn_amd/csrc/proposals.hip
@@ -16,19 +16,52 @@
     return __uint_as_float(b);
 }
 
+template <bool PLANES>
 __global__ __launch_bounds__(256)
-void rpn_decode_kernel(const float* __restrict__ head, int ld, const float* __restrict__ anchors,
-                       const float* __restrict__ valid, int A, float* __restrict__ scores,
-                       f32x4* __restrict__ boxes_all, u64* __restrict__ keys)
+void rpn_decode_kernel(float* __restrict__ head, int ld, const float* __restrict__ planes, const float* __restrict__ bias, int splits,
+                       const float* __restrict__ anchors, const float* __restrict__ valid, int A, float* __restrict__ scores,
+                       f32x4* __restrict__ boxes_all, u64* __restrict__ keys, int32_t* __restrict__ counts)
 {
     const int n = blockIdx.x * 256 + threadIdx.x;
+    if (counts != nullptr && n < 4) counts[n] = 0;
     if (n >= A) return;
     const int pix = n / 9, k = n - pix * 9;
-    const float* row = head + (size_t)pix * ld;
-    const float logit = row[k];
+    float* row = head + (size_t)pix * ld;
+    const size_t plane = (size_t)(A / 9) * 45;
+    float hv[5];
+#pragma unroll
+    for (int i = 0; i < 5; ++i) {
+        const int c = i == 0 ? k : 9 + 4 * k + (i - 1);
+        if constexpr (PLANES) hv[i] = planes[(size_t)pix * 45 + c];
+        else hv[i] = row[c];
+    }
+    if constexpr (PLANES) {
+        for (int z0 = 1; z0 < splits; z0 += 4) {
+            float t[4][5];
+#pragma unroll
+            for (int q = 0; q < 4; ++q)
+#pragma unroll
+                for (int i = 0; i < 5; ++i) {
+                    const int c = i == 0 ? k : 9 + 4 * k + (i - 1);
+                    t[q][i] = z0 + q < splits ? planes[(size_t)(z0 + q) * plane + (size_t)pix * 45 + c] : 0.f;
+                }
+#pragma unroll
+            for (int q = 0; q < 4; ++q)
+                if (z0 + q < splits) {
+#pragma unroll
+                    for (int i = 0; i < 5; ++i) hv[i] += t[q][i];
+                }
+        }
+#pragma unroll
+        for (int i = 0; i < 5; ++i) {
+            const int c = i == 0 ? k : 9 + 4 * k + (i - 1);
+            hv[i] += bias[c];
+            row[c] = hv[i];
+        }
+    }
+    const float logit = hv[0];
     const float score = 1.0f / (1.0f + expf(-logit));
-    const float dy = row[9 + 4 * k + 0], dx = row[9 + 4 * k + 1];
-    const float dh = row[9 + 4 * k + 2], dw = row[9 + 4 * k + 3];
+    const float dy = hv[1], dx = hv[2], dh = hv[3], dw = hv[4];
     const f32x4 a = reinterpret_cast<const f32x4*>(anchors)[n];
     const float cy = __fadd_rn(__fmul_rn(a[2], dy), a[0]);
     const float cx = __fadd_rn(__fmul_rn(a[3], dx), a[1]);
@@ -439,62 +472,55 @@
     }
 }
 
-__global__ __launch_bounds__(1024)
+static constexpr int EMIT_THREADS = 256;
+__global__ __launch_bounds__(EMIT_THREADS)
 void topk_emit_kernel(const f32x4* __restrict__ tmp_boxes, const float* __restrict__ tmp_scores, const int32_t* __restrict__ keep_flag,
-                      int sort_n, f32x4* __restrict__ cand_boxes, float* __restrict__ cand_scores, int32_t* __restrict__ counts)
-{
-    __shared__ int wave_tot[16];
-    const int tid = threadIdx.x;
+                      f32x4* __restrict__ cand_boxes, float* __restrict__ cand_scores, int32_t* __restrict__ counts)
+{
+    typedef int i32x4 __attribute__((ext_vector_type(4)));
+    __shared__ int wave_before[EMIT_THREADS / 64], wave_tot[EMIT_THREADS / 64];
+    const int tid = threadIdx.x, lane = tid & 63, wv = tid >> 6;
     const int n = counts[0];
-    auto body = [&](auto perc) {
-        constexpr int PER = decltype(perc)::value;
-        int fl[PER];
-        f32x4 bx[PER];
-        float sc[PER];
-#pragma unroll
-        for (int q = 0; q < PER; ++q) {
-            const int r = tid * PER + q;
-            const bool in = r < n;
-            fl[q] = in ? keep_flag[r] : 0;
-            bx[q] = in ? tmp_boxes[r] : f32x4{0.f, 0.f, 0.f, 0.f};
-            sc[q] = in ? tmp_scores[r] : 0.f;
-        }
-        int local = 0;
-#pragma unroll
-        for (int q = 0; q < PER; ++q) local += fl[q] ? 1 : 0;
-        int incl = local;
-        for (int o = 1; o < 64; o <<= 1) {
-            const int v = __shfl_up(incl, o);
-            if ((tid & 63) >= o) incl += v;
-        }
-        if ((tid & 63) == 63) wave_tot[tid >> 6] = incl;
-        __syncthreads();
-        int wave_off = 0;
-        for (int wv = 0; wv < (tid >> 6); ++wv) wave_off += wave_tot[wv];
-        int pos = wave_off + incl - local;
-#pragma unroll
-        for (int q = 0; q < PER; ++q) {
-            if (fl[q]) {
-                cand_boxes[pos] = bx[q];
-                cand_scores[pos] = sc[q];
-                ++pos;
-            }
-        }
-        if (tid == 1023) counts[1] = pos;
-    };
-    const int per = sort_n >> 10 ? sort_n >> 10 : 1;
-    if (per == 8) body(std::integral_constant<int, 8>());
-    else if (per == 16) body(std::integral_constant<int, 16>());
-    else if (per == 4) body(std::integral_constant<int, 4>());
-    else if (per == 2) body(std::integral_constant<int, 2>());
-    else body(std::integral_constant<int, 1>());
+    const int r0 = blockIdx.x * EMIT_THREADS;
+    if (r0 >= n) {
+        if (n == 0 && blockIdx.x == 0 && tid == 0) counts[1] = 0;
+        return;
+    }
+    const int r = r0 + tid;
+    const bool in = r < n;
+    const int fl = in ? (keep_flag[r] ? 1 : 0) : 0;
+    const f32x4 bx = in ? tmp_boxes[r] : f32x4{0.f, 0.f, 0.f, 0.f};
+    const float sc = in ? tmp_scores[r] : 0.f;
+    int before = 0;
+    const i32x4* f4 = reinterpret_cast<const i32x4*>(keep_flag);
+    for (int i = tid; i < (r0 >> 2); i += EMIT_THREADS) {
+        const i32x4 v = f4[i];
+        before += (v[0] ? 1 : 0) + (v[1] ? 1 : 0) + (v[2] ? 1 : 0) + (v[3] ? 1 : 0);
+    }
+    for (int o = 32; o > 0; o >>= 1) before += __shfl_xor(before, o);
+    int incl = fl;
+    for (int o = 1; o < 64; o <<= 1) {
+        const int v = __shfl_up(incl, o);
+        if (lane >= o) incl += v;
+    }
+    if (lane == 63) { wave_before[wv] = before; wave_tot[wv] = incl; }
+    __syncthreads();
+    int pos = incl - fl;
+    for (int w = 0; w < EMIT_THREADS / 64; ++w) pos += wave_before[w] + (w < wv ? wave_tot[w] : 0);
+    if (fl) {
+        cand_boxes[pos] = bx;
+        cand_scores[pos] = sc;
+    }
+    if (r == n - 1) counts[1] = pos + fl;
 }
 
 static constexpr int NMS_BAND = 32;
 
 __host__ __device__ __forceinline__ int nms_tri(int k) { return k * (k + 1) / 2; }
 
-__global__ __launch_bounds__(64)
+static constexpr int NMS_MASK_WAVES = 4;
+template <int WAVES>
+__global__ __launch_bounds__(64 * WAVES)
 void nms_mask_kernel(const f32x4* __restrict__ boxes, const int32_t* __restrict__ n_ptr, float thr,
                      int nw_stride, u64* __restrict__ mask, int bx_begin, const int32_t* __restrict__ done)
 {
@@ -507,20 +533,31 @@
     const int by = tile - nms_tri(bx);
     if (bx * 64 >= n) return;
     __shared__ f32x4 colb[64];
-    const int t = threadIdx.x;
+    __shared__ u64 part[WAVES > 1 ? (WAVES - 1) * 64 : 1];
+    const int t = threadIdx.x & 63, wv = threadIdx.x >> 6;
     const int jn = bx * 64 + t;
-    colb[t] = jn < n ? boxes[jn] : f32x4{0.f, 0.f, 0.f, 0.f};
+    if (wv == 0) colb[t] = jn < n ? boxes[jn] : f32x4{0.f, 0.f, 0.f, 0.f};
     __syncthreads();
     const int i = by * 64 + t;
-    if (i >= n) return;
-    const f32x4 a = boxes[i];
     u64 bits = 0ull;
-    const int jmax = (n - bx * 64) < 64 ? (n - bx * 64) : 64;
-    for (int j = 0; j < jmax; ++j) {
-        const int jj = bx * 64 + j;
-        if (jj > i && iou_gt(a, colb[j], thr)) bits |= 1ull << j;
-    }
-    mask[(size_t)i * nw_stride + bx] = bits;
+    if (i < n) {
+        const f32x4 a = boxes[i];
+        const int jmax = (n - bx * 64) < 64 ? (n - bx * 64) : 64;
+        constexpr int STEPS = 64 / WAVES;
+        const int jend = (wv + 1) * STEPS < jmax ? (wv + 1) * STEPS : jmax;
+        for (int j = wv * STEPS; j < jend; ++j) {
+            const int jj = bx * 64 + j;
+            if (jj > i && iou_gt(a, colb[j], thr)) bits |= 1ull << j;
+        }
+    }
+    if constexpr (WAVES > 1) {
+        if (wv > 0) part[(wv - 1) * 64 + t] = bits;
+        __syncthreads();
+        if (wv > 0) return;
+#pragma unroll
+        for (int w = 0; w < WAVES - 1; ++w) bits |= part[w * 64 + t];
+    }
+    if (i < n) mask[(size_t)i * nw_stride + bx] = bits;
 }
 
 __device__ __forceinline__ u64 readlane64(u64 v, int lane_uniform)
@@ -814,8 +851,8 @@
                            reinterpret_cast<const f32x4*>(boxes_src), ih, iw, min_side, sorted_idx, tboxes, tscores, flags);
         rc = check_launch();
         if (rc) return rc;
-        hipLaunchKernelGGL(topk_emit_kernel, dim3(1), dim3(1024), 0, s, tboxes, tscores, flags, sort_n, reinterpret_cast<f32x4*>(cand_boxes),
-                           cand_scores, counts);
+        hipLaunchKernelGGL(topk_emit_kernel, dim3(cdiv(K, EMIT_THREADS)), dim3(EMIT_THREADS), 0, s, tboxes, tscores, flags,
+                           reinterpret_cast<f32x4*>(cand_boxes), cand_scores, counts);
         return check_launch();
     }
     auto kern = topk_sort_kernel<MODE>;
@@ -835,21 +872,26 @@
     FRCNN_MAX_LDS_ONCE(nms_reduce_kernel, NMS_LDS_BYTES);
     int rc;
     if (!banded) {
-        hipLaunchKernelGGL(nms_mask_kernel, dim3(nms_tri(nw)), dim3(64), 0, s, boxes, n_ptr, thr, nw_stride, ps.mask, 0, (const int32_t*)nullptr);
+        hipLaunchKernelGGL(nms_mask_kernel<1>, dim3(nms_tri(nw)), dim3(64), 0, s, boxes, n_ptr, thr, nw_stride, ps.mask, 0, (const int32_t*)nullptr);
         rc = check_launch();
         if (rc) return rc;
         hipLaunchKernelGGL(nms_reduce_kernel, dim3(1), dim3(64), NMS_LDS_BYTES, s, ps.mask, nw_stride, n_ptr, max_keep, boxes, order, keep,
                            props, n_keep, nw, (const int32_t*)nullptr, (int32_t*)nullptr);
         return check_launch();
     }
-    hipLaunchKernelGGL(nms_mask_kernel, dim3(nms_tri(NMS_BAND)), dim3(64), 0, s, boxes, n_ptr, thr, nw_stride, ps.mask, 0, (const int32_t*)nullptr);
+    static const bool one_wave = frcnn_knob("FRCNN_NMS_MASK_ONE_WAVE") != nullptr;
+    if (one_wave)
+        hipLaunchKernelGGL(nms_mask_kernel<1>, dim3(nms_tri(NMS_BAND)), dim3(64), 0, s, boxes, n_ptr, thr, nw_stride, ps.mask, 0, (const int32_t*)nullptr);
+    else
+        hipLaunchKernelGGL(nms_mask_kernel<NMS_MASK_WAVES>, dim3(nms_tri(NMS_BAND)), dim3(64 * NMS_MASK_WAVES), 0, s, boxes, n_ptr, thr, nw_stride,
+                           ps.mask, 0, (const int32_t*)nullptr);
     rc = check_launch();
     if (rc) return rc;
     hipLaunchKernelGGL(nms_reduce_kernel, dim3(1), dim3(64), NMS_LDS_BYTES, s, ps.mask, nw_stride, n_ptr, max_keep, boxes, order, keep,
                        props, n_keep, NMS_BAND, (const int32_t*)nullptr, done);
     rc = check_launch();
     if (rc) return rc;
-    hipLaunchKernelGGL(nms_mask_kernel, dim3(nms_tri(nw) - nms_tri(NMS_BAND)), dim3(64), 0, s, boxes, n_ptr, thr, nw_stride, ps.mask, NMS_BAND,
+    hipLaunchKernelGGL(nms_mask_kernel<1>, dim3(nms_tri(nw) - nms_tri(NMS_BAND)), dim3(64), 0, s, boxes, n_ptr, thr, nw_stride, ps.mask, NMS_BAND,
                        (const int32_t*)done);
     rc = check_launch();
     if (rc) return rc;
@@ -862,14 +904,19 @@
                          const float* anchor_map, const float* valid_map, int fh, int fw,
                          int image_h, int image_w, int pre_nms, int post_nms, float nms_thr,
                          float min_side, float* scores, int32_t* sorted_idx, float* props,
-                         int32_t* counts, hipStream_t s)
+                         int32_t* counts, hipStream_t s, const HeadPlanes* planes)
 {
     const int A = fh * fw * 9;
     if (A < 1 || A > ps.a_cap || pre_nms < 1 || pre_nms > ps.pre_cap || post_nms < 1 ||
         post_nms > ps.post_cap || post_nms > 2048 || ld_head < 45)
         return FRCNN_EINVAL;
-    hipLaunchKernelGGL(rpn_decode_kernel, dim3(cdiv(A, 256)), dim3(256), 0, s, head, ld_head, anchor_map,
-                       valid_map, A, scores, reinterpret_cast<f32x4*>(ps.boxes_all), ps.keys);
+    if (planes != nullptr)
+        hipLaunchKernelGGL(rpn_decode_kernel<true>, dim3(cdiv(A, 256)), dim3(256), 0, s, planes->head_out, ld_head, planes->ws, planes->bias,
+                           planes->splits, anchor_map, valid_map, A, scores, reinterpret_cast<f32x4*>(ps.boxes_all), ps.keys, counts);
+    else
+        hipLaunchKernelGGL(rpn_decode_kernel<false>, dim3(cdiv(A, 256)), dim3(256), 0, s, const_cast<float*>(head), ld_head,
+                           (const float*)nullptr, (const float*)nullptr, 1, anchor_map, valid_map, A, scores,
+                           reinterpret_cast<f32x4*>(ps.boxes_all), ps.keys, counts);
     int rc = check_launch();
     if (rc) return rc;
     rc = launch_topk<0>(ps.keys, A, pre_nms, ps.boxes_all, (float)image_h, (float)image_w, min_side,
diff --git a/include/frcnn_hip.h b/include/frcnn_hip.h
--- a/include/frcnn_hip.h
+++ b/include/frcnn_hip.h
@@ -19,6 +19,7 @@
 
 #define FRCNN_RELU   1u
 #define FRCNN_POOL2  2u
+#define FRCNN_LINEAR_WHOLE_TILES 0x100u
 #define FRCNN_X3G_WSPLIT 0x800u
 
 int         frcnn_abi_version(void);
@@ -137,6 +138,8 @@
 int frcnn_linear(const float* d_a, int lda, const float* d_w, const float* d_bias,
                  float* d_y, int ldy, int M, int N, int K, unsigned flags,
                  void* d_ws, size_t ws_bytes, void* stream);
+int frcnn_linear_heads(const float* d_a, int lda, const float* d_w, const float* d_bias, float* d_logits, int ld, int M, int ncls,
+                       int ndelta, int K, unsigned flags, void* d_ws, size_t ws_bytes, float* d_classes, float* d_deltas, void* stream);
 int frcnn_softmax_rows(const float* d_x, int ldx, float* d_y, int M, int ncls, void* stream);
 
 typedef struct frcnn_ctx frcnn_ctx;
```

After: 992.4 (median of 6 runs). Within noise of the previous version (+0.8%).
